# uibk-uncover/ws-unet

Hardware: AMD Instinct MI355X
Metric: 512x512 grayscale images/sec (UNet predict) (higher is better)
Workload: dtype f16 MFMA on the f16 halves + ONE block-scaled fp4 (e2m1) MFMA per tap pair for both residual cross terms (per-pixel / per-(co, tap) E8M0 scales), fp32 accumulate; planar storage

## Files before the change

### ws_unet_amd/csrc/conv3x3_q.hip

```cpp
#include "wsu_device.h"
#include <cstdlib>

namespace {

constexpr int TW = 32, TH = 16, IW = TW + 2, IH = TH + 2;
constexpr int NPIX = IW * IH;
constexpr int PLANE = NPIX * 16;
constexpr int IN_SEG = (NPIX + 63) / 64;
constexpr int S_LDS = IN_SEG * 256;
constexpr int IN_SLOT = 3 * PLANE + S_LDS;
constexpr int W_GRAN = 9 * 3 * WSU_COB * 16;
constexpr int W_SLOT = W_GRAN + 1024;
constexpr int NIN = 3, NWS = 2;
constexpr int W_BASE = NIN * IN_SLOT;
constexpr int LDS_EXTRA = W_BASE + NWS * W_SLOT;
constexpr int ZERO_BYTES = 3 * IW * 16 + 32;
constexpr int LDS_TOTAL = LDS_EXTRA + 1024 * 4 + 4 * 64 * 4 + 16 + ZERO_BYTES;
static_assert(LDS_TOTAL <= 160 * 1024 && W_SLOT % 1024 == 0, "LDS budget");
constexpr int NLOAD = 4;
constexpr int W_PIECES = W_SLOT / 1024;
constexpr unsigned OOB = 0xFFFFFFF0u;
constexpr int IN_SLOT_H = 2 * PLANE;
constexpr int W_SLOT_H = 9 * 2 * WSU_COB * 16;
template <int FMT> struct QGeo {
    static_assert(FMT == WSU_PLANAR_Q || FMT == WSU_PLANAR_H, "conv3x3_q_kernel formats: Q and H");
    static constexpr bool H = FMT == WSU_PLANAR_H;
    static constexpr int in_slot = H ? IN_SLOT_H : IN_SLOT, w_slot = H ? W_SLOT_H : W_SLOT;
    static constexpr int w_planes = H ? 2 : 3;
    static constexpr int w_base = NIN * in_slot, lds_extra = w_base + NWS * w_slot;
    static constexpr int lds_zero = lds_extra + 1024 * 4 + 4 * 64 * 4 + 16;
    static constexpr int lds_total = lds_zero + (H ? 0 : ZERO_BYTES);
    static constexpr int w_pieces = w_slot / 1024;
};
static_assert(QGeo<WSU_PLANAR_Q>::lds_zero % 16 == 0 && ZERO_BYTES % 16 == 0 && ZERO_BYTES >= 3 * IW * 16 + 16 && ZERO_BYTES >= 512 + 16, "zero block");
static_assert(QGeo<WSU_PLANAR_Q>::lds_total == LDS_TOTAL && QGeo<WSU_PLANAR_Q>::w_pieces == W_PIECES && W_SLOT_H % 1024 == 0, "LDS geometry");

struct QArgs {
    const char* x1; const char* x2; const char* wp; const float* bias;
    char* y; char* ypool;
    const float* head_w; const float* head_b; float* head_out; float* head_logit; int head_cout;
    int n, h, w, c1, c2, cout;
    int tiles_x, tiles_y, ncb, nch1, nch;
    int relu;
    int ntiles;
    unsigned* range_flag;
    int msplit;
    const float* img; const float* w1; const float* b1;
};

struct Tile { int n, y0, x0, cb, mh; };
__device__ __forceinline__ Tile tile_of(const QArgs& a, int t) {
    Tile r;
    r.cb = t % a.ncb; t /= a.ncb;
    const int tx = t % a.tiles_x; t /= a.tiles_x;
    const int ty = t % a.tiles_y;
    r.n = t / a.tiles_y; r.y0 = ty * TH; r.x0 = tx * TW;
    r.mh = 0;
    if (a.msplit) { r.mh = r.cb & 1; r.cb >>= 1; }
    return r;
}

typedef __attribute__((address_space(3))) void lds_void;
typedef __attribute__((address_space(3))) char lds_char;

__device__ __forceinline__ float dpp_xor1(float v) {
    return __builtin_bit_cast(float, __builtin_amdgcn_update_dpp(0, __builtin_bit_cast(int, v), 0xB1 , 0xF, 0xF, true));
}

template <int FMT, int LW>
__device__ __forceinline__ void q_loader(const QArgs& a, char* smem, int lane, int lw, int G, int J) {
    using Gm = QGeo<FMT>;
    constexpr int NSEG = LW < 2 ? 3 : 2;
    constexpr int NIN_OPS = (Gm::H ? 2 : 4) * NSEG;
    constexpr int W0 = Gm::H ? (LW < 2 ? LW * 3 : 6 + (LW - 2) * 6) : (LW < 2 ? LW * 5 : 10 + (LW - 2) * 9);
    constexpr int NWP = Gm::H ? (LW < 2 ? 3 : 6) : (LW < 2 ? 5 : 9);
    static_assert(2 * 5 + 2 * 9 == W_PIECES && 2 * 3 + 2 * 6 == QGeo<WSU_PLANAR_H>::w_pieces, "weight pieces over the loader waves");
    lds_char* smem3 = (lds_char*)smem;
    const unsigned hw16 = (unsigned)(a.h * a.w) * 16u;
    const unsigned chunk_bytes = Gm::H ? (unsigned)wsu_h_chunk_bytes(a.h, a.w) : (unsigned)wsu_q_chunk_bytes(a.h, a.w);
    unsigned voff[NSEG], soff[NSEG];
    auto plan = [&](const Tile& t) __attribute__((always_inline)) {
        WSU_STATIC_FOR(NSEG, k, {
            const int idx = min((LW + NLOAD * k) * 64 + lane, NPIX - 1);
            const int r = idx / IW, c = idx - r * IW;
            const int yy = wsu_reflect(t.y0 - 1 + r, a.h), xx = wsu_reflect(t.x0 - 1 + c, a.w);
            voff[k] = (unsigned)(yy * a.w + xx) * 16u;
            if constexpr (!Gm::H) soff[k] = 3u * hw16 + wsu_q_soff(yy, xx, a.tiles_x);
        });
    };
    Tile ti = tile_of(a, lw); int ci = 0, kti = 0;
    int cbw = ti.cb, cw = 0, ktw = 0;
    auto issue_in = [&](int s) __attribute__((always_inline)) {
        const char* in_src = ci < a.nch1 ? a.x1 + ((size_t)ti.n * a.nch1 + ci) * chunk_bytes : a.x2 + ((size_t)ti.n * (a.nch - a.nch1) + (ci - a.nch1)) * chunk_bytes;
        const auto rs_in = __builtin_amdgcn_make_buffer_rsrc(const_cast<char*>(in_src), 0, (int)chunk_bytes, 0x00020000);
        lds_char* slot = smem3 + (s % NIN) * Gm::in_slot;
        WSU_STATIC_FOR(NSEG, k, {
            constexpr int seg = LW + NLOAD * k;
            const bool live = seg < IN_SEG - 1 || lane < NPIX - (IN_SEG - 1) * 64;
            if (live) {
                __builtin_amdgcn_raw_ptr_buffer_load_lds(rs_in, (lds_void*)(slot + seg * 1024), 16, voff[k], 0, 0, 0);
                __builtin_amdgcn_raw_ptr_buffer_load_lds(rs_in, (lds_void*)(slot + PLANE + seg * 1024), 16, voff[k], (int)hw16, 0, 0);
                if constexpr (!Gm::H) {
                    __builtin_amdgcn_raw_ptr_buffer_load_lds(rs_in, (lds_void*)(slot + 2 * PLANE + seg * 1024), 16, voff[k], (int)(2u * hw16), 0, 0);
                    __builtin_amdgcn_raw_ptr_buffer_load_lds(rs_in, (lds_void*)(slot + 3 * PLANE + seg * 256), 1, soff[k], 0, 0, 0);
                }
            }
        });
        if (++ci == a.nch && s + 1 < J) { ci = 0; ++kti; ti = tile_of(a, lw + kti * G); plan(ti); }
    };
    auto issue_w = [&](int s) __attribute__((always_inline)) {
        const auto rs_w = __builtin_amdgcn_make_buffer_rsrc(const_cast<char*>(a.wp), 0, 0x7FFFFFF0, 0x00020000);
        const int w_base = (cbw * a.nch + cw) * Gm::w_slot;
        lds_char* slot = smem3 + Gm::w_base + (s % NWS) * Gm::w_slot;
        WSU_STATIC_FOR(NWP, k, {
            constexpr int piece = W0 + k;
            __builtin_amdgcn_raw_ptr_buffer_load_lds(rs_w, (lds_void*)(slot + piece * 1024), 16, (unsigned)lane * 16u, w_base + piece * 1024, 0, 0);
        });
        if (++cw == a.nch && s + 1 < J) { cw = 0; ++ktw; cbw = tile_of(a, lw + ktw * G).cb; }
    };
    if (J <= 0) return;
    plan(ti);
    issue_w(0);
    issue_in(0);
    if (J > 1) issue_in(1);
    if (J > 1) asm volatile("s_waitcnt vmcnt(%0)" :: "n"(NIN_OPS) : "memory"); else asm volatile("s_waitcnt vmcnt(0)" ::: "memory");
    for (int j = 0; ; ++j) {
        __builtin_amdgcn_s_barrier();
        asm volatile("" ::: "memory");
        if (j + 1 >= J) break;
        issue_w(j + 1);
        const bool more = j + 2 < J;
        if (more) issue_in(j + 2);
        if (more) asm volatile("s_waitcnt vmcnt(%0)" :: "n"(NIN_OPS) : "memory"); else asm volatile("s_waitcnt vmcnt(0)" ::: "memory");
    }
}

__device__ __forceinline__ void q_loader_f1(const QArgs& a, char* smem, int lane, int lw, int G, int J, int lw8) {
    if (J <= 0) return;
    lds_char* smem3 = (lds_char*)smem;
    constexpr int F1_PX = 3;
    float pimg[F1_PX][9];
    float f1_max = 0.f;
    Tile ti = tile_of(a, lw); int ci = 0, kti = 0;
    int cbw = ti.cb, cw = 0, ktw = 0;
    auto window = [&](const Tile& tt) __attribute__((always_inline)) {
        const float* img = a.img + (size_t)tt.n * a.h * a.w;
#pragma unroll
        for (int k = 0; k < F1_PX; ++k) {
            const int idx = min((lw8 + NLOAD * k) * 64 + lane, NPIX - 1);
            const int r = idx / IW, cc = idx - r * IW;
            const int yy = wsu_reflect(tt.y0 - 1 + r, a.h), xx = wsu_reflect(tt.x0 - 1 + cc, a.w);
#pragma unroll
            for (int tp = 0; tp < 9; ++tp)
                pimg[k][tp] = img[(size_t)wsu_reflect(yy + tp / 3 - 1, a.h) * a.w + wsu_reflect(xx + tp % 3 - 1, a.w)];
        }
    };
    typedef __attribute__((address_space(4))) const f32x2 cst_f32x2;
    auto compute_in = [&](int s) __attribute__((always_inline)) {
        char* slot = smem + (s % NIN) * IN_SLOT;
        cst_f32x2* wt = (cst_f32x2*)(a.w1 + ci * 16);
        cst_f32x2* bt = (cst_f32x2*)(a.b1 + ci * 16);
        f32x2 acc[F1_PX][8];
#pragma unroll
        for (int g = 0; g < 8; ++g) {
            const f32x2 b = bt[g];
#pragma unroll
            for (int k = 0; k < F1_PX; ++k) acc[k][g] = b;
        }
#pragma unroll
        for (int tp = 0; tp < 9; ++tp) {
            f32x2 wv[8];
#pragma unroll
            for (int g = 0; g < 8; ++g) wv[g] = wt[tp * 32 + g];
#pragma unroll
            for (int k = 0; k < F1_PX; ++k) {
                const f32x2 pw = {pimg[k][tp & ~1], pimg[k][(tp | 1) < 9 ? (tp | 1) : tp]};
#pragma unroll
                for (int g = 0; g < 8; ++g) {
                    if (tp & 1) asm volatile("v_pk_fma_f32 %0, %1, %2, %0 op_sel:[1,0,0] op_sel_hi:[1,1,1]" : "+v"(acc[k][g]) : "v"(pw), "s"(wv[g]));
                    else asm volatile("v_pk_fma_f32 %0, %1, %2, %0 op_sel:[0,0,0] op_sel_hi:[0,1,1]" : "+v"(acc[k][g]) : "v"(pw), "s"(wv[g]));
                }
            }
        }
        asm volatile("s_nop 0" ::: "memory");
#pragma unroll
        for (int k = 0; k < F1_PX; ++k) {
            const int idx = (lw8 + NLOAD * k) * 64 + lane;
            f32x4 v[4];
#pragma unroll
            for (int g = 0; g < 4; ++g) v[g] = mk_f4(acc[k][2 * g][0], acc[k][2 * g][1], acc[k][2 * g + 1][0], acc[k][2 * g + 1][1]);
#pragma unroll
            for (int g = 0; g < 4; ++g)
#pragma unroll
                for (int e = 0; e < 4; ++e) { v[g][e] = fmaxf(v[g][e], 0.f); f1_max = fmaxf(f1_max, v[g][e]); }
            u32x4 h0, h1, qg; uint32_t sb;
            wsu_q4_encode16(v, h0, h1, qg, sb);
            if (lw8 + NLOAD * k < IN_SEG && idx < NPIX) {
                char* d = slot + idx * 16;
                *reinterpret_cast<u32x4*>(d) = h0;
                *reinterpret_cast<u32x4*>(d + PLANE) = h1;
                *reinterpret_cast<u32x4*>(d + 2 * PLANE) = qg;
                *reinterpret_cast<uint32_t*>(slot + 3 * PLANE + idx * 4) = sb;
            }
        }
        if (++ci == a.nch && s + 1 < J) { ci = 0; ++kti; ti = tile_of(a, lw + kti * G); window(ti); }
    };
    const int w0 = lw8 < 2 ? lw8 * 5 : 10 + (lw8 - 2) * 9, nwp = lw8 < 2 ? 5 : 9;
    auto issue_w = [&](int s) __attribute__((always_inline)) {
        const auto rs_w = __builtin_amdgcn_make_buffer_rsrc(const_cast<char*>(a.wp), 0, 0x7FFFFFF0, 0x00020000);
        const int w_base = (cbw * a.nch + cw) * W_SLOT;
        lds_char* slot = smem3 + W_BASE + (s % NWS) * W_SLOT;
#pragma unroll
        for (int k = 0; k < 9; ++k)
            if (k < nwp)
                __builtin_amdgcn_raw_ptr_buffer_load_lds(rs_w, (lds_void*)(slot + (w0 + k) * 1024), 16, (unsigned)lane * 16u, w_base + (w0 + k) * 1024, 0, 0);
        if (++cw == a.nch && s + 1 < J) { cw = 0; ++ktw; cbw = tile_of(a, lw + ktw * G).cb; }
    };
    window(ti);
    issue_w(0);
    compute_in(0);
    if (J > 1) compute_in(1);
    asm volatile("s_waitcnt vmcnt(0) lgkmcnt(0)" ::: "memory");
    for (int j = 0; ; ++j) {
        __builtin_amdgcn_s_barrier();
        asm volatile("" ::: "memory");
        if (j + 1 >= J) break;
        issue_w(j + 1);
        if (j + 2 < J) compute_in(j + 2);
        asm volatile("s_waitcnt vmcnt(0) lgkmcnt(0)" ::: "memory");
    }
    if (a.range_flag && __builtin_amdgcn_ballot_w64(!(f1_max <= WSU_F8_RANGE)) != 0 && lane == 0) atomicOr(a.range_flag, 1u);
}

template <int RQ, int HC, bool POOL, bool FQ, bool MSPLIT, bool F1 = false, int FMT = WSU_PLANAR_Q>
__global__ __launch_bounds__((16 / RQ + NLOAD) * 64) __attribute__((amdgpu_waves_per_eu(RQ == 4 ? 2 : 3, RQ == 4 ? 2 : 3)))
void conv3x3_q_kernel(const QArgs a) {
    using Gm = QGeo<FMT>;
    constexpr bool H = Gm::H;
    static_assert(!(H && F1), "the fused first layer computes Q inputs");
    constexpr int NWAVE = 16 / RQ, NT = (NWAVE + NLOAD) * 64;
    extern __shared__ __attribute__((aligned(16))) char smem[];
    const int tid = threadIdx.x;
    const int wv = __builtin_amdgcn_readfirstlane(tid >> 6), lane = tid & 63, l31 = lane & 31, hh = lane >> 5;
    const int l31_k = l31, hh_k = hh;
    const int G = gridDim.x;
    const int lw = (int)wsu_xcd_remap(blockIdx.x, G);
    const int K = a.ntiles > lw ? (a.ntiles - lw + G - 1) / G : 0;
    const int J = K * a.nch;

    float* s_bias = reinterpret_cast<float*>(smem + Gm::lds_extra);
    float* s_hw = s_bias + 1024;
    float* s_hb = s_hw + 4 * 64;
    for (int i = tid; i < a.cout; i += NT) s_bias[i] = a.bias ? a.bias[i] : 0.f;
    constexpr bool HEAD = HC > 0;
    if constexpr (HEAD) {
        for (int i = tid; i < a.head_cout * 64; i += NT) s_hw[i] = a.head_w[i];
        if (tid < 4) s_hb[tid] = (a.head_b && tid < a.head_cout) ? a.head_b[tid] : 0.f;
    }
    if constexpr (!Gm::H) {
        for (int i = tid; i < ZERO_BYTES / 4; i += NT) reinterpret_cast<unsigned*>(smem + Gm::lds_zero)[i] = 0u;
        asm volatile("s_waitcnt lgkmcnt(0)" ::: "memory");
    }

    if (wv >= NWAVE) {
        if constexpr (F1) { q_loader_f1(a, smem, lane, lw, G, J, wv - NWAVE); return; }
        switch (wv - NWAVE) {
            case 0: q_loader<FMT, 0>(a, smem, lane, lw, G, J); break;
            case 1: q_loader<FMT, 1>(a, smem, lane, lw, G, J); break;
            case 2: q_loader<FMT, 2>(a, smem, lane, lw, G, J); break;
            default: q_loader<FMT, 3>(a, smem, lane, lw, G, J); break;
        }
        return;
    }

    Tile cur = tile_of(a, lw);
    constexpr int MH = MSPLIT ? 1 : 2;
    constexpr bool PIPE = !H;
    constexpr bool EPO = !MSPLIT && HC == 0 && RQ != 4;
    f32x16 acc[2][4];
    int kt = 0, j = 0;
    unsigned q_in_off = 0, q_w_off = Gm::w_base;
    unsigned nx_in = 0, nx_w = Gm::w_base;
    unsigned a_off = 0, b_off = 0, x_w = 0, x_w4 = 0, x_sa = 0, x_sa4 = 0, x_b1 = 0, x_b2 = 0, x_b4 = 0, x_sb0 = 0, x_sb1 = 0, x_sb2 = 0;
    constexpr unsigned W4_IMM = (unsigned)((8 * 3 + 2) * 64) * 16u, B4_IMM = (unsigned)(2 * IW + 2) * 16u;
    typedef __attribute__((address_space(3))) const unsigned char lds_cuchar;
    typedef __attribute__((address_space(3))) const int lds_cint;
    typedef __attribute__((address_space(3))) const u32x4 lds_cu32x4;
    const unsigned Lb = (unsigned)(size_t)(lds_char*)smem;
    auto at = [](unsigned addr) __attribute__((always_inline)) { return (lds_char*)(size_t)addr; };
    auto begin_step = [&]() __attribute__((always_inline)) {
        q_in_off = nx_in; q_w_off = nx_w;
        nx_in = nx_in + (unsigned)Gm::in_slot == (unsigned)(NIN * Gm::in_slot) ? 0u : nx_in + (unsigned)Gm::in_slot;
        static_assert(NWS == 2, "nx_w toggles between the two weight slots the loaders fill as s % NWS");
        nx_w = (unsigned)(2 * Gm::w_base + Gm::w_slot) - nx_w;
        a_off = Lb + q_w_off + (unsigned)((cur.mh * 32 + l31) * 16) + (unsigned)(hh * 64 * 16);
        b_off = Lb + q_in_off + (unsigned)(((RQ * wv) * IW + l31) * 16) + (unsigned)(hh * PLANE);
        if constexpr (!H) {
            unsigned hq = (unsigned)hh;
            asm volatile("" : "+v"(hq));
            const unsigned zero = Lb + (unsigned)Gm::lds_zero;
            const unsigned w0 = Lb + q_w_off + (unsigned)(cur.mh * 32 + l31) * 16u;
            const unsigned p0 = Lb + q_in_off + 2 * PLANE + (unsigned)((RQ * wv) * IW + l31) * 16u;
            x_w = w0 + hq * (unsigned)(3 * 64 * 16);
            x_w4 = hq ? zero - W4_IMM : w0;
            x_sa4 = Lb + q_w_off + W_GRAN + (unsigned)(cur.mh * 32 + l31);
            x_sa = x_sa4 + hq * 64u;
            x_b1 = p0 + hq * 16u;
            x_b2 = p0 + hq * (unsigned)((IW - 2) * 16);
            x_b4 = hq ? zero - B4_IMM : p0;
            x_sb0 = Lb + q_in_off + 3 * PLANE + (unsigned)((RQ * wv) * IW + l31) * 4u;
            x_sb1 = x_sb0 + hq * 4u;
            x_sb2 = x_sb0 + hq * (unsigned)((IW - 2) * 4);
            asm volatile("" : "+v"(a_off), "+v"(b_off), "+v"(x_w), "+v"(x_w4), "+v"(x_sa), "+v"(x_sa4));
            asm volatile("" : "+v"(x_b1), "+v"(x_b2), "+v"(x_b4), "+v"(x_sb0), "+v"(x_sb1), "+v"(x_sb2));
        } else {
            asm volatile("" : "+v"(a_off), "+v"(b_off));
        }
        __builtin_amdgcn_s_barrier();
        asm volatile("" ::: "memory");
    };
    auto zero_acc = [&]() __attribute__((always_inline)) {
#pragma unroll
        for (int m = 0; m < MH; ++m)
#pragma unroll
            for (int q = 0; q < RQ; ++q)
#pragma unroll
                for (int r = 0; r < 16; ++r) acc[m][q][r] = 0.f;
    };
    auto main_term = [&](auto tap_c, auto ms_c, auto first_c) __attribute__((always_inline)) {
        constexpr int tap = decltype(tap_c)::value, dy = tap / 3, dx = tap % 3;
        constexpr int ms = decltype(ms_c)::value, ML = ms < 0 ? 0 : ms, MU = ms < 0 ? MH : ms + 1;
        constexpr bool FIRST = decltype(first_c)::value;
        u32x4 ah[2], bh[4];
_Pragma("unroll")
        for (int m = ML; m < MU; ++m) ah[m] = *(lds_cu32x4*)(at(a_off) + ((tap * Gm::w_planes) * 64 + m * 32) * 16);
_Pragma("unroll")
        for (int q = 0; q < RQ; ++q) bh[q] = *(lds_cu32x4*)(at(b_off) + ((q + dy) * IW + dx) * 16);
_Pragma("unroll")
        for (int m = ML; m < MU; ++m)
_Pragma("unroll")
            for (int q = 0; q < RQ; ++q) {
                if constexpr (FIRST) acc[m][q] = wsu_mfma_f16_z(ah[m], bh[q]);
                else wsu_mfma_f16(ah[m], bh[q], acc[m][q]);
            }
    };
    auto q4_reads = [&](auto tp_c, auto ml_c, auto mu_c, u32x4* a4, u32x4* b4, int* sa, int* sb) __attribute__((always_inline)) {
        constexpr int tp = decltype(tp_c)::value, ML = decltype(ml_c)::value, MU = decltype(mu_c)::value;
        constexpr bool single = 2 * tp + 1 >= 9;
        constexpr int t0 = 2 * tp, pix0 = (t0 / 3) * IW + t0 % 3;
        constexpr unsigned wimm = (unsigned)((6 * tp + 2) * 64) * 16u;
        static_assert(!single || (wimm == W4_IMM && (unsigned)pix0 * 16u == B4_IMM), "tap 8");
        const unsigned wbase = single ? x_w4 : x_w, sabase = single ? x_sa4 : x_sa;
        const unsigned bbase = single ? x_b4 : (tp == 1 ? x_b2 : x_b1), sbbase = single ? x_sb0 : (tp == 1 ? x_sb2 : x_sb1);
_Pragma("unroll")
        for (int m = ML; m < MU; ++m) {
            a4[m] = *(lds_cu32x4*)(at(wbase) + wimm + m * 32 * 16);
            sa[m] = *(lds_cuchar*)(at(sabase) + 128 * tp + m * 32);
        }
_Pragma("unroll")
        for (int q = 0; q < RQ; ++q) {
            b4[q] = *(lds_cu32x4*)(at(bbase) + (pix0 + q * IW) * 16);
            sb[q] = *(lds_cint*)(at(sbbase) + (pix0 + q * IW) * 4);
        }
    };
    auto cross_q4 = [&](auto tp_c, auto ms_c, auto first_c) __attribute__((always_inline)) {
        constexpr int ms = decltype(ms_c)::value, ML = ms < 0 ? 0 : ms, MU = ms < 0 ? MH : ms + 1;
        constexpr bool FIRST = decltype(first_c)::value;
        u32x4 a4[2], b4[4]; int sa[2], sb[4];
        q4_reads(tp_c, std::integral_constant<int, ML>{}, std::integral_constant<int, MU>{}, a4, b4, sa, sb);
_Pragma("unroll")
        for (int m = ML; m < MU; ++m)
_Pragma("unroll")
            for (int q = 0; q < RQ; ++q) {
                if constexpr (FIRST) acc[m][q] = wsu_mfma_q4_z(a4[m], b4[q], sa[m], sb[q]);
                else wsu_mfma_q4(a4[m], b4[q], sa[m], sb[q], acc[m][q]);
            }
    };
    constexpr std::false_type not_first{};
    constexpr std::true_type tile_first{};
    auto units_range = [&](auto ms_c, auto lo_c, auto hi_c, auto first_c) __attribute__((always_inline)) {
        constexpr int lo = decltype(lo_c)::value, hi = decltype(hi_c)::value;
        constexpr bool FIRST = decltype(first_c)::value;
        static_assert(!FIRST || lo == 0, "a tile opens with tap pair 0");
        WSU_STATIC_FOR(hi - lo, i, {
            constexpr int tp = lo + i;
            if constexpr (!H) cross_q4(std::integral_constant<int, tp>{}, ms_c, std::integral_constant<bool, FIRST && tp == 0>{});
            main_term(std::integral_constant<int, 2 * tp>{}, ms_c, std::integral_constant<bool, FIRST && H && tp == 0>{});
            if constexpr (2 * tp + 1 < 9) main_term(std::integral_constant<int, 2 * tp + 1>{}, ms_c, not_first);
        });
    };
    constexpr std::integral_constant<int, -1> all_m{};
    struct Frag { u32x4 a[2]; u32x4 b[4]; int sa[2]; int sb[4]; };
    auto load_unit = [&](auto u_c, Frag& f, u32x4* row1) __attribute__((always_inline)) {
        constexpr int u = decltype(u_c)::value, tp = u / 3, k = u % 3;
        if constexpr (k == 0) {
            q4_reads(std::integral_constant<int, tp>{}, std::integral_constant<int, 0>{}, std::integral_constant<int, MH>{}, f.a, f.b, f.sa, f.sb);
        } else {
            constexpr int tap = 2 * tp + k - 1, dy = tap / 3, dx = tap % 3;
_Pragma("unroll")
            for (int m = 0; m < MH; ++m) f.a[m] = *(lds_cu32x4*)(at(a_off) + ((tap * 3) * 64 + m * 32) * 16);
            if constexpr (RQ == 2) {
                if constexpr (dy > 0) f.b[0] = row1[tap - 3];
                else f.b[0] = *(lds_cu32x4*)(at(b_off) + (dy * IW + dx) * 16);
                f.b[1] = row1[tap] = *(lds_cu32x4*)(at(b_off) + ((1 + dy) * IW + dx) * 16);
            } else {
_Pragma("unroll")
                for (int q = 0; q < RQ; ++q) f.b[q] = *(lds_cu32x4*)(at(b_off) + ((q + dy) * IW + dx) * 16);
            }
        }
    };
    auto mma_unit = [&](auto u_c, Frag& f, auto first_c) __attribute__((always_inline)) {
        constexpr int u = decltype(u_c)::value, k = u % 3;
        constexpr bool FIRST = decltype(first_c)::value && u == 0;
        if constexpr (k == 0) {
_Pragma("unroll")
            for (int m = 0; m < MH; ++m)
_Pragma("unroll")
                for (int q = 0; q < RQ; ++q) {
                    if constexpr (FIRST) acc[m][q] = wsu_mfma_q4_z(f.a[m], f.b[q], f.sa[m], f.sb[q]);
                    else wsu_mfma_q4(f.a[m], f.b[q], f.sa[m], f.sb[q], acc[m][q]);
                }
        } else {
_Pragma("unroll")
            for (int m = 0; m < MH; ++m)
_Pragma("unroll")
                for (int q = 0; q < RQ; ++q) wsu_mfma_f16(f.a[m], f.b[q], acc[m][q]);
        }
    };
    auto units_pipelined = [&](auto first_c) __attribute__((always_inline)) {
        constexpr int NU = 14;
        Frag fr[2];
        u32x4 row1[9];
        load_unit(std::integral_constant<int, 0>{}, fr[0], row1);
        WSU_STATIC_FOR(NU, u, {
            if constexpr (u + 1 < NU) load_unit(std::integral_constant<int, u + 1>{}, fr[(u + 1) % 2], row1);
            __builtin_amdgcn_sched_barrier(0);
            mma_unit(u_c, fr[u % 2], first_c);
            __builtin_amdgcn_sched_barrier(0);
        });
    };
    auto units_all = [&](auto ms_c, auto first_c) __attribute__((always_inline)) {
        if constexpr (PIPE && decltype(ms_c)::value < 0) { units_pipelined(first_c); return; }
        units_range(ms_c, std::integral_constant<int, 0>{}, std::integral_constant<int, 5>{}, first_c);
    };

    auto finish_tile = [&]() __attribute__((always_inline)) {
        int l31 = l31_k, hh = hh_k;
        asm volatile("" : "+v"(l31), "+v"(hh));
        const int col = cur.x0 + l31;
        const unsigned hw16 = (unsigned)(a.h * a.w) * 16u;
        const int nco = a.cout >> 4;
        float hz[4][HC > 0 ? HC : 1];
        float vmax = 0.f;
        const float relu_floor = a.relu ? 0.f : -__builtin_inff();
#pragma unroll
        for (int q = 0; q < RQ; ++q)
#pragma unroll
            for (int o = 0; o < (HC > 0 ? HC : 1); ++o) hz[q][o] = 0.f;
        struct QOff { unsigned g0, g1, q, s; };
        auto pair_off = [&](unsigned plane_bytes, unsigned off0, unsigned off1, unsigned soff0, unsigned soff1, bool ok0, bool ok1) __attribute__((always_inline)) {
            const unsigned hp = hh ? plane_bytes : 0u;
            const bool okm = hh ? ok1 : ok0;
            QOff o = {ok0 ? off0 + hp : OOB, ok1 ? off1 + hp : OOB, okm ? (hh ? off1 : off0) + 2u * plane_bytes : OOB, okm ? 3u * plane_bytes + (hh ? soff1 : soff0) : OOB};
            asm volatile("" : "+v"(o.g0), "+v"(o.g1), "+v"(o.q), "+v"(o.s));
            return o;
        };
        constexpr bool YQ = FQ && !H;
        QOff qo[RQ / 2] = {}, qop = {};
        if constexpr (YQ) {
            const unsigned sblk = (unsigned)(((cur.y0 >> 4) * a.tiles_x + (cur.x0 >> 5)) * 512);
_Pragma("unroll")
            for (int rp = 0; rp < RQ / 2; ++rp) {
                const int r0 = RQ * wv + 2 * rp, row0 = cur.y0 + r0;
                qo[rp] = pair_off(hw16, (unsigned)(row0 * a.w + col) * 16u, (unsigned)((row0 + 1) * a.w + col) * 16u,
                                  sblk + (unsigned)(r0 * 32 + l31), sblk + (unsigned)((r0 + 1) * 32 + l31), row0 < a.h && col < a.w, row0 + 1 < a.h && col < a.w);
            }
            if constexpr (POOL) {
                const int hp = a.h >> 1, wp2 = a.w >> 1, ptx = (wp2 + 31) >> 5;
                const int gy0 = (cur.y0 >> 1) + (RQ / 2) * wv, gx = (cur.x0 >> 1) + (l31 >> 1);
                const unsigned php16 = (unsigned)(hp * wp2) * 16u;
                if constexpr (RQ == 4) {
                    const bool okx = !(l31 & 1) && gx < wp2;
                    qop = pair_off(php16, (unsigned)(gy0 * wp2 + gx) * 16u, (unsigned)((gy0 + 1) * wp2 + gx) * 16u,
                                   wsu_q_soff(gy0, gx, ptx), wsu_q_soff(gy0 + 1, gx, ptx), okx && gy0 < hp, okx && gy0 + 1 < hp);
                } else {
                    const unsigned coff = (l31 & 1) ? (unsigned)wsu_q_chunk_bytes(hp, wp2) : 0u;
                    const unsigned off = (unsigned)(gy0 * wp2 + gx) * 16u + coff, soff = wsu_q_soff(gy0, gx, ptx) + coff;
                    const bool ok = gx < wp2 && gy0 < hp;
                    qop = {ok ? off + (hh ? php16 : 0u) : OOB, OOB, (ok && !hh) ? off + 2u * php16 : OOB, (ok && !hh) ? 3u * php16 + soff : OOB};
                    asm volatile("" : "+v"(qop.g0), "+v"(qop.q), "+v"(qop.s));
                }
            }
        }
        auto store_pair_q = [&](const f32x4& X0, const f32x4& Y0, const f32x4& X1, const f32x4& Y1, char* base, unsigned chunk_bytes, const QOff& o, bool have, bool fold) __attribute__((always_inline)) {
            u32x4 g0, g1; uint32_t dh0, dr0, sb0, dh1, dr1, sb1;
            const float mx0 = wsu_q4_pre(X0, Y0, g0, dh0, dr0, sb0);
            const float mx1 = wsu_q4_pre(X1, Y1, g1, dh1, dr1, sb1);
            if (fold) vmax = wsu_max3(vmax, mx0, mx1);
            const u32x4 qg = wsu_q4_pair(dh0, dr0, dh1, dr1);
            const auto rs = __builtin_amdgcn_make_buffer_rsrc(base, 0, have ? (int)chunk_bytes : 0, 0x00020000);
            __builtin_amdgcn_raw_buffer_store_b128(g0, rs, (int)o.g0, 0, 0);
            __builtin_amdgcn_raw_buffer_store_b128(g1, rs, (int)o.g1, 0, 0);
            __builtin_amdgcn_raw_buffer_store_b128(qg, rs, (int)o.q, 0, 0);
            __builtin_amdgcn_raw_buffer_store_b8((unsigned char)(hh ? sb1 : sb0), rs, (int)o.s, 0, 0);
        };
        auto store_one_q = [&](const f32x4& X, const f32x4& Y, char* base, unsigned chunk_bytes, const QOff& o) __attribute__((always_inline)) {
            u32x4 g; uint32_t dh, dr, sb;
            wsu_q4_pre(X, Y, g, dh, dr, sb);
            const u32x4 qg = wsu_q4_single(dh, dr);
            const auto rs = __builtin_amdgcn_make_buffer_rsrc(base, 0, (int)chunk_bytes, 0x00020000);
            __builtin_amdgcn_raw_buffer_store_b128(g, rs, (int)o.g0, 0, 0);
            __builtin_amdgcn_raw_buffer_store_b128(qg, rs, (int)o.q, 0, 0);
            __builtin_amdgcn_raw_buffer_store_b8((unsigned char)sb, rs, (int)o.s, 0, 0);
        };
        auto store_one_h = [&](const f32x4& X, const f32x4& Y, char* base, unsigned plane_bytes, unsigned off, bool ok, bool have) __attribute__((always_inline)) {
            const auto rs = __builtin_amdgcn_make_buffer_rsrc(base, 0, have ? (int)(2u * plane_bytes) : 0, 0x00020000);
            __builtin_amdgcn_raw_buffer_store_b128(wsu_h_granule(X, Y), rs, (int)(ok ? off + (hh ? plane_bytes : 0u) : OOB), 0, 0);
        };
        auto store_one_a = [&](const f32x4& X, const f32x4& Y, char* base, unsigned plane_bytes, unsigned off, bool ok, bool have) __attribute__((always_inline)) {
            uint32_t xh0, xh1, xlo, yh0, yh1, ylo;
            wsu_split4_f16r8(X, WSU_F8_XLO_DIV, xh0, xh1, xlo);
            wsu_split4_f16r8(Y, WSU_F8_XLO_DIV, yh0, yh1, ylo);
            wsu_swap32(xh0, yh0); wsu_swap32(xh1, yh1);
            uint32_t xlp = xlo, ylp = ylo;
            wsu_swap32(xlo, xlp); wsu_swap32(ylo, ylp);
            const auto rs = __builtin_amdgcn_make_buffer_rsrc(base, 0, have ? (int)(3u * plane_bytes) : 0, 0x00020000);
            __builtin_amdgcn_raw_buffer_store_b128(mk_u4(xh0, xh1, yh0, yh1), rs, (int)(ok ? off + (hh ? plane_bytes : 0u) : OOB), 0, 0);
            __builtin_amdgcn_raw_buffer_store_b128(mk_u4(xlo, xlp, ylo, ylp), rs, (int)((ok && !hh) ? off + 2u * plane_bytes : OOB), 0, 0);
        };
        auto epi_m = [&](auto m_c, auto&& hook) __attribute__((always_inline)) {
            constexpr int m = decltype(m_c)::value;
            constexpr int NH = RQ / 2;
            f32x4 spx, spy;
            auto piece = [&](auto cp_c) __attribute__((always_inline)) {
                constexpr int cp = decltype(cp_c)::value;
                const int oc = cur.cb * 4 + (m + cur.mh) * 2 + cp;
                const int co0 = oc * 16 + 4 * hh;
                const bool have_y = a.y != nullptr;
                f32x4 px[2], py[2];
                WSU_STATIC_FOR(RQ / 2, rp, {
                    hook(std::integral_constant<int, NH * cp + rp>{});
                    f32x4 vx[2], vy[2];
                    const f32x4 bx = *reinterpret_cast<const f32x4*>(s_bias + co0), by = *reinterpret_cast<const f32x4*>(s_bias + co0 + 8);
_Pragma("unroll")
                    for (int u = 0; u < 2; ++u) {
_Pragma("unroll")
                        for (int e = 0; e < 4; ++e) {
                            const float x = fmaxf(acc[m][2 * rp + u][8 * cp + e] + bx[e], relu_floor), y = fmaxf(acc[m][2 * rp + u][8 * cp + 4 + e] + by[e], relu_floor);
                            vx[u][e] = x; vy[u][e] = y;
                            if constexpr (H || !FQ) vmax = fmaxf(fmaxf(vmax, fabsf(x)), fabsf(y));
                        }
                    }
                    if constexpr (HEAD) {
                        const int lc = (m * 2 + cp) * 16 + 4 * hh;
_Pragma("unroll")
                        for (int o = 0; o < HC; ++o)
                            if (HC == 1 || o < a.head_cout)
_Pragma("unroll")
                                for (int u = 0; u < 2; ++u)
_Pragma("unroll")
                                    for (int e = 0; e < 4; ++e)
                                        hz[2 * rp + u][o] = fmaf(vx[u][e], s_hw[o * 64 + lc + e], fmaf(vy[u][e], s_hw[o * 64 + lc + 8 + e], hz[2 * rp + u][o]));
                    }
                    const int r0 = RQ * wv + 2 * rp, row0 = cur.y0 + r0;
                    if (!HEAD || have_y) {
                        if constexpr (H) {
                            char* base = a.y + ((size_t)cur.n * nco + oc) * (2u * hw16);
                            WSU_STATIC_FOR(2, u, {
                                store_one_h(vx[u], vy[u], base, hw16, (unsigned)((row0 + u) * a.w + col) * 16u, row0 + u < a.h && col < a.w, have_y);
                            });
                        } else if constexpr (FQ) {
                            const unsigned cb_ = (unsigned)wsu_q_chunk_bytes(a.h, a.w);
                            char* base = a.y + ((size_t)cur.n * nco + oc) * cb_;
                            store_pair_q(vx[0], vy[0], vx[1], vy[1], base, cb_, qo[rp], have_y, true);
                        } else {
                            char* base = a.y + (((size_t)cur.n * nco + oc) * 3) * hw16;
                            WSU_STATIC_FOR(2, u, {
                                store_one_a(vx[u], vy[u], base, hw16, (unsigned)((row0 + u) * a.w + col) * 16u, row0 + u < a.h && col < a.w, have_y);
                            });
                        }
                    }
                    if constexpr (POOL) {
_Pragma("unroll")
                        for (int e = 0; e < 4; ++e) {
                            const float cx = fmaxf(vx[0][e], vx[1][e]), cy = fmaxf(vy[0][e], vy[1][e]);
                            px[rp][e] = fmaxf(cx, dpp_xor1(cx)); py[rp][e] = fmaxf(cy, dpp_xor1(cy));
                        }
                    }
                });
                if constexpr (POOL) {
                    const int hp = a.h >> 1, wp2 = a.w >> 1;
                    const int gy0 = (cur.y0 >> 1) + (RQ / 2) * wv, gx = (cur.x0 >> 1) + (l31 >> 1);
                    const bool okx = !(l31 & 1) && gx < wp2;
                    const unsigned php16 = (unsigned)(hp * wp2) * 16u;
                    if constexpr (H) {
                        char* base = a.ypool + ((size_t)cur.n * nco + oc) * (2u * php16);
#pragma unroll
                        for (int rp = 0; rp < RQ / 2; ++rp)
                            store_one_h(px[rp], py[rp], base, php16, (unsigned)((gy0 + rp) * wp2 + gx) * 16u, okx && gy0 + rp < hp, true);
                    } else if constexpr (FQ) {
                        const unsigned cbp = (unsigned)wsu_q_chunk_bytes(hp, wp2);
                        char* base = a.ypool + ((size_t)cur.n * nco + oc) * cbp;
                        if constexpr (RQ == 4) {
                            store_pair_q(px[0], py[0], px[1], py[1], base, cbp, qop, true, false);
                        } else if constexpr (cp == 0) {
                            spx = px[0]; spy = py[0];
                        } else {
                            static_assert(cp == 1, "piece 1 closes the pair: its chunk follows piece 0's");
                            const bool odd = (l31 & 1) != 0;
                            f32x4 sx, sy;
_Pragma("unroll")
                            for (int e = 0; e < 4; ++e) { sx[e] = odd ? px[0][e] : spx[e]; sy[e] = odd ? py[0][e] : spy[e]; }
                            store_one_q(sx, sy, base - cbp, 2u * cbp, qop);
                        }
                    } else {
                        char* base = a.ypool + (((size_t)cur.n * nco + oc) * 3) * php16;
#pragma unroll
                        for (int rp = 0; rp < RQ / 2; ++rp)
                            store_one_a(px[rp], py[rp], base, php16, (unsigned)((gy0 + rp) * wp2 + gx) * 16u, okx && gy0 + rp < hp, true);
                    }
                }
            };
            piece(std::integral_constant<int, 0>{});
            piece(std::integral_constant<int, 1>{});
        };
        auto nothing = [](auto) __attribute__((always_inline)) {};
        if constexpr (EPO) {
            constexpr int NHT = 2 * (RQ / 2);
            epi_m(std::integral_constant<int, 0>{}, [&](auto h_c) __attribute__((always_inline)) {
                constexpr int h = decltype(h_c)::value;
                constexpr int lo = 5 * h / NHT, hi = 5 * (h + 1) / NHT;
                if constexpr (hi > lo) units_range(std::integral_constant<int, 1>{}, std::integral_constant<int, lo>{}, std::integral_constant<int, hi>{}, not_first);
            });
            epi_m(std::integral_constant<int, 1>{}, nothing);
        } else {
            WSU_STATIC_FOR(MH, m, { (void)m; epi_m(m_c, nothing); });
        }
        if constexpr (HEAD) {
            const size_t hw = (size_t)a.h * a.w;
#pragma unroll
            for (int q = 0; q < RQ; ++q) {
                const int row = cur.y0 + RQ * wv + q;
#pragma unroll
                for (int o = 0; o < HC; ++o)
                    if (HC == 1 || o < a.head_cout) {
                        uint32_t mine = __builtin_bit_cast(uint32_t, hz[q][o]), other = mine;
                        wsu_swap32(mine, other);
                        const float z = __builtin_bit_cast(float, mine) + __builtin_bit_cast(float, other) + s_hb[o];
                        if (!hh && row < a.h && col < a.w) {
                            const size_t plane = ((size_t)cur.n * a.head_cout + o) * hw;
                            const uint32_t off = (uint32_t)(row * a.w + col);
                            if (a.head_logit) (a.head_logit + plane)[off] = z;
                            (a.head_out + plane)[off] = 1.f / (1.f + expf(-z));
                        }
                    }
            }
        }
        if (a.range_flag && (a.y || POOL) && __builtin_amdgcn_ballot_w64(!(vmax <= (H ? WSU_F16_RANGE : WSU_F8_RANGE))) != 0 && lane == 0)
            atomicOr(a.range_flag, 1u);
        ++kt;
        if (j + 1 < J) cur = tile_of(a, lw + kt * G);
    };
    for (int t = 0; t < K; ++t) {
        if (a.nch == 1) {
            zero_acc();
        } else {
            begin_step(); units_all(all_m, tile_first); ++j;
            for (int cc = 2; cc < a.nch; ++cc) { begin_step(); units_all(all_m, not_first); ++j; }
        }
        begin_step();
        if constexpr (EPO) units_all(std::integral_constant<int, 0>{}, not_first);
        else units_all(all_m, not_first);
        __builtin_amdgcn_sched_barrier(0);
        finish_tile();
        ++j;
    }
}

__global__ void pack_conv3x3_f4_kernel(const float* __restrict__ w, char* __restrict__ dst, int cin, int cout) {
    const int nch = cin / 16;
    const long long total = (long long)(cout / WSU_COB) * nch * 9 * WSU_COB;
    for (long long d = (long long)blockIdx.x * blockDim.x + threadIdx.x; d < total; d += (long long)gridDim.x * blockDim.x) {
        long long t = d;
        const int co = (int)(t % WSU_COB); t /= WSU_COB;
        const int tap = (int)(t % 9); t /= 9;
        const int c = (int)(t % nch); const int cb = (int)(t / nch);
        float v[16], r[16];
        uint32_t h[8];
#pragma unroll
        for (int e = 0; e < 16; ++e) v[e] = w[(((size_t)(cb * WSU_COB + co) * cin + c * 16 + e) * 3 + tap / 3) * 3 + tap % 3];
#pragma unroll
        for (int e = 0; e < 8; ++e) {
            const _Float16 a = (_Float16)v[2 * e], b = (_Float16)v[2 * e + 1];
            h[e] = (uint32_t)__builtin_bit_cast(unsigned short, a) | ((uint32_t)__builtin_bit_cast(unsigned short, b) << 16);
            r[2 * e] = (v[2 * e] - (float)a) * 2048.f; r[2 * e + 1] = (v[2 * e + 1] - (float)b) * 2048.f;
        }
        const u32x4 h0 = mk_u4(h[0], h[1], h[2], h[3]), h1 = mk_u4(h[4], h[5], h[6], h[7]);
        const int E = wsu_q4_block_exp(wsu_f16x16_max_abs_bits(h0, h1));
        const float sc = wsu_pow2f(E);
        uint32_t q[4] = {0, 0, 0, 0};
        WSU_STATIC_FOR(8, e, { q[e >> 2] = __builtin_amdgcn_cvt_scalef32_pk_fp4_f32(q[e >> 2], r[2 * e], r[2 * e + 1], sc, e & 3); });
        q[2] = wsu_f16x8_to_fp4(h0, sc); q[3] = wsu_f16x8_to_fp4(h1, sc);
        char* slice = dst + ((size_t)cb * nch + c) * W_SLOT;
        char* base = slice + (size_t)(tap * 3) * (WSU_COB * 16) + co * 16;
        *reinterpret_cast<u32x4*>(base) = h0;
        *reinterpret_cast<u32x4*>(base + WSU_COB * 16) = h1;
        *reinterpret_cast<u32x4*>(base + 2 * WSU_COB * 16) = mk_u4(q[0], q[1], q[2], q[3]);
        slice[W_GRAN + tap * 64 + co] = (char)(E + 127 - 11);
        if (tap == 0 && co < 7) *reinterpret_cast<u32x4*>(slice + W_GRAN + 576 + co * 64) = mk_u4(0, 0, 0, 0), *reinterpret_cast<u32x4*>(slice + W_GRAN + 576 + co * 64 + 16) = mk_u4(0, 0, 0, 0),
            *reinterpret_cast<u32x4*>(slice + W_GRAN + 576 + co * 64 + 32) = mk_u4(0, 0, 0, 0), *reinterpret_cast<u32x4*>(slice + W_GRAN + 576 + co * 64 + 48) = mk_u4(0, 0, 0, 0);
    }
}

__global__ void pack_conv3x3_h_kernel(const float* __restrict__ w, char* __restrict__ dst, int cin, int cout) {
    const int nch = cin / 16;
    const long long total = (long long)(cout / WSU_COB) * nch * 9 * WSU_COB;
    for (long long d = (long long)blockIdx.x * blockDim.x + threadIdx.x; d < total; d += (long long)gridDim.x * blockDim.x) {
        long long t = d;
        const int co = (int)(t % WSU_COB); t /= WSU_COB;
        const int tap = (int)(t % 9); t /= 9;
        const int c = (int)(t % nch); const int cb = (int)(t / nch);
        uint32_t h[8];
#pragma unroll
        for (int e = 0; e < 8; ++e) {
            const size_t i0 = (((size_t)(cb * WSU_COB + co) * cin + c * 16 + 2 * e) * 3 + tap / 3) * 3 + tap % 3;
            const _Float16 a = (_Float16)w[i0], b = (_Float16)w[i0 + 9];
            h[e] = (uint32_t)__builtin_bit_cast(unsigned short, a) | ((uint32_t)__builtin_bit_cast(unsigned short, b) << 16);
        }
        char* base = dst + ((size_t)cb * nch + c) * W_SLOT_H + (size_t)(tap * 2) * (WSU_COB * 16) + co * 16;
        *reinterpret_cast<u32x4*>(base) = mk_u4(h[0], h[1], h[2], h[3]);
        *reinterpret_cast<u32x4*>(base + WSU_COB * 16) = mk_u4(h[4], h[5], h[6], h[7]);
    }
}

#define WSU_Q_VARIANTS_RQ(X, RQ)                    \
    X(RQ, 0, false, false, false, false, WSU_PLANAR_Q) \
    X(RQ, 0, false, true, false, false, WSU_PLANAR_Q)  \
    X(RQ, 0, true, false, false, false, WSU_PLANAR_Q)  \
    X(RQ, 0, true, true, false, false, WSU_PLANAR_Q)   \
    X(RQ, 1, false, false, false, false, WSU_PLANAR_Q) \
    X(RQ, 4, false, false, false, false, WSU_PLANAR_Q) \
    X(RQ, 0, false, false, true, false, WSU_PLANAR_Q)  \
    X(RQ, 0, false, true, true, false, WSU_PLANAR_Q)
#define WSU_Q_VARIANTS(X)                            \
    WSU_Q_VARIANTS_RQ(X, 4)                          \
    WSU_Q_VARIANTS_RQ(X, 2)                          \
    X(2, 0, true, true, false, true, WSU_PLANAR_Q)   \
    X(2, 0, false, true, false, false, WSU_PLANAR_H) \
    X(2, 0, true, true, false, false, WSU_PLANAR_H)  \
    X(2, 1, false, true, false, false, WSU_PLANAR_H) \
    X(2, 4, false, true, false, false, WSU_PLANAR_H) \
    X(2, 0, false, true, true, false, WSU_PLANAR_H)
#define WSU_Q_INST(RQ, HC, POOL, FQ, MSPLIT, F1, FMT) template __global__ void conv3x3_q_kernel<RQ, HC, POOL, FQ, MSPLIT, F1, FMT>(const QArgs);
WSU_Q_VARIANTS(WSU_Q_INST)

struct QVariant {
    int rq, hc; bool pool, fq, msplit, f1; int fmt;
    void (*kernel)(const QArgs);
    bool raised;
};
#define WSU_Q_ROW(RQ, HC, POOL, FQ, MSPLIT, F1, FMT) {RQ, HC, POOL, FQ, MSPLIT, F1, FMT, conv3x3_q_kernel<RQ, HC, POOL, FQ, MSPLIT, F1, FMT>, false},
QVariant q_variants[] = {WSU_Q_VARIANTS(WSU_Q_ROW)};

int q_launch(QArgs a, const char* who, int fmt, int rq, bool yq, bool msplit_on, hipStream_t s) {
    const bool h = fmt == WSU_PLANAR_H, f1 = a.img != nullptr;
    const int ncu = wsu_cu_count(who);
    if (!ncu) return WSU_ERR_HIP;
    const int hc = !a.head_w ? 0 : (a.head_cout == 1 ? 1 : 4);
    const bool pool = a.ypool != nullptr, fq = h || (yq && !hc);
    a.msplit = !f1 && msplit_on && !hc && !pool && 2 * (long long)a.ntiles <= ncu;
    if (a.msplit) { a.ncb *= 2; a.ntiles *= 2; }
    for (QVariant& v : q_variants) {
        if (v.rq != rq || v.hc != hc || v.pool != pool || v.fq != fq || v.msplit != (a.msplit != 0) || v.f1 != f1 || v.fmt != fmt) continue;
        const int lds = h ? QGeo<WSU_PLANAR_H>::lds_total : LDS_TOTAL;
        if (!v.raised) {
            if (int rc = wsu_raise_lds(v.kernel, lds, f1 ? "conv3x3_q<F1>" : (h ? "conv3x3_q<H>" : "conv3x3_q"))) return rc;
            v.raised = true;
        }
        hipLaunchKernelGGL(v.kernel, dim3(a.ntiles < ncu ? a.ntiles : ncu), dim3((16 / rq + NLOAD) * 64), lds, s, a);
        return wsu_check_launch(f1 ? "conv3x3_q_kernel<F1>" : (h ? (a.msplit ? "conv3x3_q_kernel<H, msplit>" : "conv3x3_q_kernel<H>")
                                                                 : (a.msplit ? "conv3x3_q_kernel<msplit>" : "conv3x3_q_kernel")));
    }
    wsu_set_error("%s: no kernel variant for this combination of outputs", who);
    return WSU_ERR_UNSUPPORTED;
}

int q_args(QArgs& a, const char* who, const void* x1, const void* x2, const float* img, const float* w1, const float* b1, const void* wp, const float* bias,
           void* y, void* y_pool, const float* head_w, const float* head_b, float* head_out, float* head_logit, int head_cout,
           int n, int h, int w, int c1, int c2, int cout, int relu, int y_format, unsigned formats, const char* formats_msg, unsigned* range_flag) {
    const bool f1 = img || w1 || b1;
    WSU_REQUIRE(wp && (f1 ? img && w1 && b1 && y && y_pool : x1 && (y || y_pool || head_w)), "%s: null pointer", who);
    WSU_REQUIRE(!f1 || (((uintptr_t)w1 & 63) == 0 && ((uintptr_t)b1 & 63) == 0), "%s: w1_taps and b1 must be 64-byte aligned (scalar 16-dword loads)", who);
    WSU_REQUIRE(y_format >= 0 && y_format < 32 && ((formats >> y_format) & 1u), "%s: y_format must be %s", who, formats_msg);
    WSU_REQUIRE(n > 0 && h >= 2 && w >= 2, "%s: bad shape n=%d h=%d w=%d (reflect pad 1 needs h,w >= 2)", who, n, h, w);
    WSU_REQUIRE(c1 > 0 && c1 % 16 == 0 && c2 >= 0 && c2 % 16 == 0 && (c2 == 0) == (x2 == nullptr), "%s: c1=%d c2=%d must be multiples of 16", who, c1, c2);
    WSU_REQUIRE(cout > 0 && cout % WSU_COB == 0 && cout <= 1024, "%s: cout=%d must be a multiple of %d (<= 1024)", who, cout, WSU_COB);
    WSU_REQUIRE(!head_w || (head_out && cout == WSU_COB && head_cout >= 1 && head_cout <= 4), "%s: fused head needs cout == %d and 1..4 head planes", who, WSU_COB);
    WSU_REQUIRE(!y_pool || (h % 2 == 0 && w % 2 == 0), "%s: fused pool needs even h, w (got h=%d w=%d)", who, h, w);
    WSU_REQUIRE(!(y_pool && head_w), "%s: the fused pool and the fused head exclude each other", who);
    WSU_REQUIRE(!(head_w && y && y_format == WSU_PLANAR_Q), "%s: a y beside the fused head is written in format WSU_PLANAR_A", who);
    WSU_REQUIRE((long long)h * w * 50 < 0xFFFFFFF0LL, "%s: h*w too large (a chunk must stay below 4 GiB)", who);
    a.x1 = (const char*)x1; a.x2 = (const char*)x2; a.wp = (const char*)wp; a.bias = bias;
    a.y = (char*)y; a.ypool = (char*)y_pool;
    a.head_w = head_w; a.head_b = head_b; a.head_out = head_out; a.head_logit = head_logit; a.head_cout = head_cout;
    a.range_flag = range_flag;
    a.n = n; a.h = h; a.w = w; a.c1 = c1; a.c2 = c2; a.cout = cout;
    a.tiles_x = (w + TW - 1) / TW; a.tiles_y = (h + TH - 1) / TH; a.ncb = cout / WSU_COB;
    a.nch1 = c1 / 16; a.nch = (c1 + c2) / 16; a.relu = relu; a.msplit = 0;
    a.img = img; a.w1 = w1; a.b1 = b1;
    const long long nt = (long long)n * a.tiles_x * a.tiles_y * a.ncb;
    WSU_REQUIRE(nt > 0 && nt < 0x3FFFFFFFLL, "%s: %lld tiles out of range", who, nt);
    a.ntiles = (int)nt;
    return WSU_OK;
}

bool q_msplit_on() {
    static const int on = [] { const char* e = getenv("WSU_PL_MSPLIT"); return e ? atoi(e) : 1; }();
    return on != 0;
}

size_t packed_bytes(int cin, int cout, int slot) {
    if (cin <= 0 || cout <= 0 || cin % 16 || cout % WSU_COB) return 0;
    return (size_t)(cout / WSU_COB) * (cin / 16) * slot;
}
int pack(void (*kernel)(const float*, char*, int, int), const char* who, const char* kernel_name, const float* w_oihw, void* w_packed, int cin, int cout, void* stream) {
    WSU_REQUIRE(w_oihw && w_packed, "%s: null pointer", who);
    WSU_REQUIRE(cin > 0 && cin % 16 == 0 && cout > 0 && cout % WSU_COB == 0, "%s: cin=%d must be a multiple of 16, cout=%d of %d", who, cin, cout, WSU_COB);
    hipLaunchKernelGGL(kernel, dim3(512), dim3(256), 0, static_cast<hipStream_t>(stream), w_oihw, (char*)w_packed, cin, cout);
    return wsu_check_launch(kernel_name);
}

}

extern "C" {

size_t wsu_conv3x3_packed_f4_bytes(int cin, int cout) { return packed_bytes(cin, cout, W_SLOT); }
int wsu_conv3x3_pack_f4(const float* w_oihw, void* w_packed, int cin, int cout, void* stream) {
    return pack(pack_conv3x3_f4_kernel, "conv3x3_pack_f4", "pack_conv3x3_f4_kernel", w_oihw, w_packed, cin, cout, stream);
}

int wsu_conv3x3_q_fused_first_fwd(const float* img, const float* w1_taps, const float* b1, const void* w_packed_f4, const float* bias, void* y, void* y_pool,
                                  int n, int h, int w, int cout, int relu, unsigned* range_flag, void* stream) {
    const char* who = "conv3x3_q_fused_first";
    WSU_REQUIRE(img && w1_taps && b1, "%s: null pointer", who);
    QArgs a;
    if (int rc = q_args(a, who, nullptr, nullptr, img, w1_taps, b1, w_packed_f4, bias, y, y_pool, nullptr, nullptr, nullptr, nullptr, 0,
                        n, h, w, 64, 0, cout, relu, WSU_PLANAR_Q, 1u << WSU_PLANAR_Q, "WSU_PLANAR_Q", range_flag)) return rc;
    return q_launch(a, who, WSU_PLANAR_Q, 2, true, false, static_cast<hipStream_t>(stream));
}

size_t wsu_planar_q_bytes(int n, int c, int h, int w) {
    if (n <= 0 || c <= 0 || c % 16 || h <= 0 || w <= 0) return 0;
    return (size_t)n * (size_t)(c / 16) * wsu_q_chunk_bytes(h, w);
}

int wsu_conv3x3_q_fwd(const void* x1, const void* x2, const void* w_packed_f4, const float* bias, void* y, void* y_pool,
                      const float* head_w, const float* head_b, float* head_out, float* head_logit, int head_cout,
                      int n, int h, int w, int c1, int c2, int cout, int relu, int y_format, unsigned* range_flag, void* stream) {
    QArgs a;
    if (int rc = q_args(a, "conv3x3_q", x1, x2, nullptr, nullptr, nullptr, w_packed_f4, bias, y, y_pool, head_w, head_b, head_out, head_logit, head_cout,
                        n, h, w, c1, c2, cout, relu, y_format, 1u << WSU_PLANAR_A | 1u << WSU_PLANAR_Q, "WSU_PLANAR_A or WSU_PLANAR_Q", range_flag)) return rc;
    static const int rq = [] { const char* e = getenv("WSU_Q_ROWS"); return (e && atoi(e) == 4) ? 4 : 2; }();
    return q_launch(a, "conv3x3_q", WSU_PLANAR_Q, rq, y_format == WSU_PLANAR_Q, q_msplit_on(), static_cast<hipStream_t>(stream));
}

size_t wsu_planar_h_bytes(int n, int c, int h, int w) {
    if (n <= 0 || c <= 0 || c % 16 || h <= 0 || w <= 0) return 0;
    return (size_t)n * (size_t)(c / 16) * wsu_h_chunk_bytes(h, w);
}

size_t wsu_conv3x3_packed_h_bytes(int cin, int cout) { return packed_bytes(cin, cout, W_SLOT_H); }
int wsu_conv3x3_pack_h(const float* w_oihw, void* w_packed, int cin, int cout, void* stream) {
    return pack(pack_conv3x3_h_kernel, "conv3x3_pack_h", "pack_conv3x3_h_kernel", w_oihw, w_packed, cin, cout, stream);
}

int wsu_conv3x3_h_fwd(const void* x1, const void* x2, const void* w_packed_h, const float* bias, void* y, void* y_pool,
                      const float* head_w, const float* head_b, float* head_out, float* head_logit, int head_cout,
                      int n, int h, int w, int c1, int c2, int cout, int relu, int y_format, unsigned* range_flag, void* stream) {
    QArgs a;
    if (int rc = q_args(a, "conv3x3_h", x1, x2, nullptr, nullptr, nullptr, w_packed_h, bias, y, y_pool, head_w, head_b, head_out, head_logit, head_cout,
                        n, h, w, c1, c2, cout, relu, y_format, 1u << WSU_PLANAR_H, "WSU_PLANAR_H", range_flag)) return rc;
    return q_launch(a, "conv3x3_h", WSU_PLANAR_H, 2, true, q_msplit_on(), static_cast<hipStream_t>(stream));
}

}
```

### ws_unet_amd/csrc/conv3x3_qu.hip

```cpp
#include "wsu_device.h"

namespace {

constexpr int TW = 32, TH = 16;
constexpr int CW = 17, CH = 9, CPIX = CW * CH;
constexpr int NPIX_S = 4 * CPIX;
constexpr int PLANE_S = NPIX_S * 16;
constexpr int SEG_S = (NPIX_S + 63) / 64;
constexpr int IN_S = 3 * PLANE_S + SEG_S * 256;
constexpr int LP = 33, LH = TH / 2 + 2, LW_ = TW / 2 + 2;
constexpr int NPIX_L = LP * LH;
constexpr int PLANE_L = NPIX_L * 16;
constexpr int SEG_L = (NPIX_L + 63) / 64;
constexpr int IN_L = 3 * PLANE_L + SEG_L * 256;
constexpr int W_GRAN_S = 9 * 3 * WSU_COB * 16;
constexpr int W_S = W_GRAN_S + 1024;
constexpr int W_UNITS_L = 8;
constexpr int W_GRAN_L = W_UNITS_L * 3 * WSU_COB * 16;
constexpr int W_L = W_GRAN_L + 1024;
constexpr int PIECES_S = W_S / 1024, PIECES_L = W_L / 1024;
constexpr int REGION = 80640;
constexpr int OFF_SW = IN_S, OFF_LIN = W_L, OFF_LW1 = W_L + IN_L;
constexpr int LDS_BIAS = 2 * REGION;
constexpr int MAX_COUT = 512;
constexpr int LDS_TOTAL = LDS_BIAS + MAX_COUT * 4;
static_assert(IN_S + W_S <= REGION && OFF_LW1 + W_L <= REGION && (REGION & 0xF) == 0 && LDS_TOTAL <= 160 * 1024, "LDS budget");
static_assert((OFF_SW | OFF_LIN | OFF_LW1) % 16 == 0, "16-byte aligned allocations");
constexpr int ZERO_BYTES = 576;
constexpr int LDS_ZERO = 2 * REGION - ZERO_BYTES;
static_assert(IN_S + W_S <= REGION - ZERO_BYTES && OFF_LW1 + W_L <= REGION - ZERO_BYTES && LDS_ZERO % 16 == 0 && ZERO_BYTES >= 2 * CW * 16 + 16 + 16, "zero block");
constexpr int NLOAD = 4, NWAVE = 8, NT = (NWAVE + NLOAD) * 64;
constexpr unsigned OOB = 0xFFFFFFF0u;
constexpr int W_S_H = 9 * 2 * WSU_COB * 16;
constexpr int W_L_H = W_UNITS_L * 2 * WSU_COB * 16;
constexpr int PIECES_S_H = W_S_H / 1024, PIECES_L_H = W_L_H / 1024;

struct UArgs {
    const char* xl; const char* xs; const char* wps; const char* wpl; const float* bias;
    char* y;
    int n, h, w, hl, wl, cl, c2, cout;
    int tiles_x, tiles_y, ltiles_x, ncb, nchS, nchL;
    int relu, ntiles;
    unsigned* range_flag;
};

struct Tile { int n, y0, x0, cb; };
__device__ __forceinline__ Tile tile_of(const UArgs& a, int t) {
    Tile r;
    r.cb = t % a.ncb; t /= a.ncb;
    const int tx = t % a.tiles_x; t /= a.tiles_x;
    const int ty = t % a.tiles_y;
    r.n = t / a.tiles_y; r.y0 = ty * TH; r.x0 = tx * TW;
    return r;
}

typedef __attribute__((address_space(3))) void lds_void;
typedef __attribute__((address_space(3))) char lds_char;

__device__ __forceinline__ void wait_vm(int n) {
#define WSU_VM_CASE(k) case k: asm volatile("s_waitcnt vmcnt(" #k ")" ::: "memory"); break;
    switch (n) {
        WSU_VM_CASE(0) WSU_VM_CASE(1) WSU_VM_CASE(2) WSU_VM_CASE(3) WSU_VM_CASE(4) WSU_VM_CASE(5) WSU_VM_CASE(6) WSU_VM_CASE(7) WSU_VM_CASE(8) WSU_VM_CASE(9)
        WSU_VM_CASE(10) WSU_VM_CASE(11) WSU_VM_CASE(12) WSU_VM_CASE(13) WSU_VM_CASE(14) WSU_VM_CASE(15) WSU_VM_CASE(16) WSU_VM_CASE(17) WSU_VM_CASE(18) WSU_VM_CASE(19)
        WSU_VM_CASE(20) WSU_VM_CASE(21) WSU_VM_CASE(22) WSU_VM_CASE(23) WSU_VM_CASE(24) WSU_VM_CASE(25) WSU_VM_CASE(26) WSU_VM_CASE(27) WSU_VM_CASE(28) WSU_VM_CASE(29)
        WSU_VM_CASE(30) WSU_VM_CASE(31) WSU_VM_CASE(32) WSU_VM_CASE(33) WSU_VM_CASE(34) WSU_VM_CASE(35) WSU_VM_CASE(36) WSU_VM_CASE(37) WSU_VM_CASE(38) WSU_VM_CASE(39)
        default: asm volatile("s_waitcnt vmcnt(0)" ::: "memory"); break;
    }
#undef WSU_VM_CASE
}


template <int FMT, int LW>
__device__ __forceinline__ void u_loader(const UArgs& a, char* smem, int lane, int lw, int G, int K) {
    constexpr bool H = FMT == WSU_PLANAR_H;
    constexpr int NSS = LW < 2 ? 3 : 2;
    constexpr int NSL = LW < 2 ? 2 : 1;
    constexpr int OPS_INS = (H ? 2 : 4) * NSS, OPS_INL = (H ? 2 : 4) * NSL;
    constexpr int WS0 = H ? (LW < 2 ? LW * 3 : 6 + (LW - 2) * 6) : (LW < 2 ? LW * 5 : 10 + (LW - 2) * 9);
    constexpr int NWS = H ? (LW < 2 ? 3 : 6) : (LW < 2 ? 5 : 9);
    constexpr int WL0 = H ? (LW < 2 ? LW * 3 : 6 + (LW - 2) * 5) : (LW < 2 ? LW * 5 : (LW == 2 ? 10 : 17));
    constexpr int NWL = H ? (LW < 2 ? 3 : 5) : (LW < 2 ? 5 : (LW == 2 ? 7 : 8));
    constexpr int WSLICE_S = H ? W_S_H : W_S, WSLICE_L = H ? W_L_H : W_L;
    static_assert(2 * 5 + 2 * 9 == PIECES_S && 2 * 5 + 7 + 8 == PIECES_L, "weight pieces over the loader waves");
    static_assert(2 * 3 + 2 * 6 == PIECES_S_H && 2 * 3 + 2 * 5 == PIECES_L_H, "weight pieces over the loader waves (format H)");
    lds_char* smem3 = (lds_char*)smem;
    const unsigned hw16 = (unsigned)(a.h * a.w) * 16u, hwl16 = (unsigned)(a.hl * a.wl) * 16u;
    const unsigned cbytes_s = H ? (unsigned)wsu_h_chunk_bytes(a.h, a.w) : (unsigned)wsu_q_chunk_bytes(a.h, a.w);
    const unsigned cbytes_l = H ? (unsigned)wsu_h_chunk_bytes(a.hl, a.wl) : (unsigned)wsu_q_chunk_bytes(a.hl, a.wl);
    const int T = a.nchS + a.nchL;
    const int J = K * T;
    if (J <= 0) return;
    unsigned voS[NSS], soS[NSS], voL[NSL], soL[NSL];
    auto plan = [&](const Tile& t) __attribute__((always_inline)) {
        WSU_STATIC_FOR(NSS, k, {
            const int idx = min((LW + NLOAD * k) * 64 + lane, NPIX_S - 1);
            const int p = idx / CPIX, rem = idx - p * CPIX;
            const int lr = rem / CW, lc = rem - lr * CW;
            const int yy = wsu_reflect(t.y0 - 1 + 2 * lr + (p >> 1), a.h), xx = wsu_reflect(t.x0 - 1 + 2 * lc + (p & 1), a.w);
            voS[k] = (unsigned)(yy * a.w + xx) * 16u;
            if constexpr (!H) soS[k] = 3u * hw16 + wsu_q_soff(yy, xx, a.tiles_x);
        });
        WSU_STATIC_FOR(NSL, k, {
            const int idx = min((LW + NLOAD * k) * 64 + lane, NPIX_L - 1);
            const int r = idx / LP, c = min(idx - r * LP, LW_ - 1);
            const int yy = min(max((t.y0 >> 1) - 1 + r, 0), a.hl - 1), xx = min(max((t.x0 >> 1) - 1 + c, 0), a.wl - 1);
            voL[k] = (unsigned)(yy * a.wl + xx) * 16u;
            if constexpr (!H) soL[k] = 3u * hwl16 + wsu_q_soff(yy, xx, a.ltiles_x);
        });
    };
    int a_kt = 0, a_c = 0, a_r = 0; bool a_low = false;
    Tile at = tile_of(a, lw);
    unsigned region = 0;
    auto issue_alloc = [&](lds_char* slot) __attribute__((always_inline)) {
        int nops;
        const bool is_in = a_low ? a_r == 1 : a_r == 0;
        if (is_in && !a_low) {
            const char* src = a.xs + ((size_t)at.n * a.nchS + a_c) * cbytes_s;
            const auto rs = __builtin_amdgcn_make_buffer_rsrc(const_cast<char*>(src), 0, (int)cbytes_s, 0x00020000);
            WSU_STATIC_FOR(NSS, k, {
                constexpr int seg = LW + NLOAD * k;
                if (seg < SEG_S - 1 || lane < NPIX_S - (SEG_S - 1) * 64) {
                    __builtin_amdgcn_raw_ptr_buffer_load_lds(rs, (lds_void*)(slot + seg * 1024), 16, voS[k], 0, 0, 0);
                    __builtin_amdgcn_raw_ptr_buffer_load_lds(rs, (lds_void*)(slot + PLANE_S + seg * 1024), 16, voS[k], (int)hw16, 0, 0);
                    if constexpr (!H) {
                        __builtin_amdgcn_raw_ptr_buffer_load_lds(rs, (lds_void*)(slot + 2 * PLANE_S + seg * 1024), 16, voS[k], (int)(2u * hw16), 0, 0);
                        __builtin_amdgcn_raw_ptr_buffer_load_lds(rs, (lds_void*)(slot + 3 * PLANE_S + seg * 256), 1, soS[k], 0, 0, 0);
                    }
                }
            });
            nops = OPS_INS;
        } else if (is_in) {
            const char* src = a.xl + ((size_t)at.n * a.nchL + a_c) * cbytes_l;
            const auto rs = __builtin_amdgcn_make_buffer_rsrc(const_cast<char*>(src), 0, (int)cbytes_l, 0x00020000);
            WSU_STATIC_FOR(NSL, k, {
                constexpr int seg = LW + NLOAD * k;
                if (seg < SEG_L - 1 || lane < NPIX_L - (SEG_L - 1) * 64) {
                    __builtin_amdgcn_raw_ptr_buffer_load_lds(rs, (lds_void*)(slot + seg * 1024), 16, voL[k], 0, 0, 0);
                    __builtin_amdgcn_raw_ptr_buffer_load_lds(rs, (lds_void*)(slot + PLANE_L + seg * 1024), 16, voL[k], (int)hwl16, 0, 0);
                    if constexpr (!H) {
                        __builtin_amdgcn_raw_ptr_buffer_load_lds(rs, (lds_void*)(slot + 2 * PLANE_L + seg * 1024), 16, voL[k], (int)(2u * hwl16), 0, 0);
                        __builtin_amdgcn_raw_ptr_buffer_load_lds(rs, (lds_void*)(slot + 3 * PLANE_L + seg * 256), 1, soL[k], 0, 0, 0);
                    }
                }
            });
            nops = OPS_INL;
        } else if (!a_low) {
            const auto rs = __builtin_amdgcn_make_buffer_rsrc(const_cast<char*>(a.wps), 0, 0x7FFFFFF0, 0x00020000);
            const int base = (at.cb * a.nchS + a_c) * WSLICE_S;
            WSU_STATIC_FOR(NWS, k, {
                constexpr int piece = WS0 + k;
                __builtin_amdgcn_raw_ptr_buffer_load_lds(rs, (lds_void*)(slot + piece * 1024), 16, (unsigned)lane * 16u, base + piece * 1024, 0, 0);
            });
            nops = NWS;
        } else {
            const auto rs = __builtin_amdgcn_make_buffer_rsrc(const_cast<char*>(a.wpl), 0, 0x7FFFFFF0, 0x00020000);
            const int base = ((at.cb * a.nchL + a_c) * 2 + (a_r == 2 ? 1 : 0)) * WSLICE_L;
            WSU_STATIC_FOR(NWL, k, {
                constexpr int piece = WL0 + k;
                __builtin_amdgcn_raw_ptr_buffer_load_lds(rs, (lds_void*)(slot + piece * 1024), 16, (unsigned)lane * 16u, base + piece * 1024, 0, 0);
            });
            nops = NWL;
        }
        return nops;
    };
    auto issue_step = [&]() __attribute__((always_inline)) {
        lds_char* base = smem3 + region;
        int nops;
        if (!a_low) {
            a_r = 0; nops = issue_alloc(base);
            a_r = 1; nops += issue_alloc(base + OFF_SW);
            if (++a_c == a.nchS) { a_c = 0; a_low = true; }
        } else {
            a_r = 0; nops = issue_alloc(base);
            a_r = 1; nops += issue_alloc(base + OFF_LIN);
            a_r = 2; nops += issue_alloc(base + OFF_LW1);
            if (++a_c == a.nchL) {
                a_low = false; a_c = 0;
                if (++a_kt < K) { at = tile_of(a, lw + a_kt * G); plan(at); }
            }
        }
        region ^= (unsigned)REGION;
        return nops;
    };
    plan(at);
    {
        issue_step();
        const int n1 = J > 1 ? issue_step() : 0;
        wait_vm(n1);
    }
    for (int j = 0; ; ++j) {
        __builtin_amdgcn_s_barrier();
        asm volatile("" ::: "memory");
        if (j + 1 >= J) break;
        if (j >= 1) issue_step();
        wait_vm(0);
    }
}

template <int FMT>
__global__ __launch_bounds__(NT) __attribute__((amdgpu_waves_per_eu(3, 3)))
void conv3x3_qu_kernel(const UArgs a) {
    constexpr bool H = FMT == WSU_PLANAR_H;
    constexpr int WPL = H ? 2 : 3;
    extern __shared__ __attribute__((aligned(16))) char smem[];
    const int tid = threadIdx.x;
    const int wv = __builtin_amdgcn_readfirstlane(tid >> 6), lane = tid & 63;
    const int G = gridDim.x;
    const int lw = (int)wsu_xcd_remap(blockIdx.x, G);
    const int K = a.ntiles > lw ? (a.ntiles - lw + G - 1) / G : 0;
    float* s_bias = reinterpret_cast<float*>(smem + LDS_BIAS);
    for (int i = tid; i < a.cout; i += NT) s_bias[i] = a.bias ? a.bias[i] : 0.f;
    if constexpr (!H) {
        for (int i = tid; i < ZERO_BYTES / 4; i += NT) reinterpret_cast<unsigned*>(smem + LDS_ZERO)[i] = 0u;
        asm volatile("s_waitcnt lgkmcnt(0)" ::: "memory");
    }

    if (wv >= NWAVE) {
        switch (wv - NWAVE) {
            case 0: u_loader<FMT, 0>(a, smem, lane, lw, G, K); break;
            case 1: u_loader<FMT, 1>(a, smem, lane, lw, G, K); break;
            case 2: u_loader<FMT, 2>(a, smem, lane, lw, G, K); break;
            default: u_loader<FMT, 3>(a, smem, lane, lw, G, K); break;
        }
        return;
    }

    const int cls = wv & 3, py = cls >> 1, px = cls & 1, rh = wv >> 2;
    const int l31 = lane & 31, hh = lane >> 5;
    const int lrow = l31 >> 4, lcol = lrow ? ((l31 + 15) & 15) : l31;
    const unsigned laneS = (unsigned)(((4 * rh + lrow) * CW + lcol) * 16), laneL = (unsigned)(((4 * rh + lrow) * LP + lcol) * 16);
    constexpr unsigned QS = 2 * CW * 16, QL = 2 * LP * 16;
    Tile cur = tile_of(a, lw);
    f32x16 acc[2][2];
    unsigned region = 0;
    unsigned in_off = 0, w_off = 0;
    auto next_region = [&]() __attribute__((always_inline)) { const unsigned r = region; region ^= (unsigned)REGION; return r; };
    int hh_q = hh;
    typedef __attribute__((address_space(3))) const unsigned char lds_cuchar;
    typedef __attribute__((address_space(3))) const int lds_cint;
    typedef __attribute__((address_space(3))) const u32x4 lds_cu32x4;
    lds_char* L = (lds_char*)smem;
    const unsigned Lb = (unsigned)(size_t)L;
    auto at = [](unsigned addr) __attribute__((always_inline)) { return (lds_char*)(size_t)addr; };
    auto tap_s = [&](int ky, int kx) __attribute__((always_inline)) {
        return (unsigned)(((((py + ky) & 1) * 2 + ((px + kx) & 1)) * CPIX + ((py + ky) >> 1) * CW + ((px + kx) >> 1)) * 16);
    };
    unsigned a_off = 0, b_off = 0, hd_w = 0, hd_sa = 0, hd_b = 0, hd_sb = 0, x_w = 0, x_w4 = 0, x_sa = 0, x_sa4 = 0, x_b4 = 0;
    constexpr unsigned W4_IMM = (unsigned)((8 * 3 + 2) * 64) * 16u;
    unsigned tap_sel[5] = {};
    if constexpr (!H) {
        WSU_STATIC_FOR(5, tp, {
            constexpr int t0 = 2 * tp, t1 = (2 * tp + 1 < 9) ? 2 * tp + 1 : 2 * tp;
            tap_sel[tp] = ((hh ? tap_s(t1 / 3, t1 % 3) : tap_s(t0 / 3, t0 % 3)) + laneS) >> 2;
            asm volatile("" : "+v"(tap_sel[tp]));
        });
    }
    auto sync_step = [&](auto low_c) __attribute__((always_inline)) {
        constexpr bool LOW = decltype(low_c)::value;
        const unsigned r = next_region();
        in_off = LOW ? r + OFF_LIN : r;
        w_off = LOW ? r : r + OFF_SW;
        hh_q = hh;
        asm volatile("" : "+v"(hh_q));
        a_off = Lb + w_off + (unsigned)l31 * 16u + (unsigned)hh * 1024u;
        b_off = Lb + in_off + (unsigned)hh * (LOW ? PLANE_L : PLANE_S) + (LOW ? laneL : laneS);
        if constexpr (!H && !LOW) {
            const unsigned hq = (unsigned)hh_q, zero = Lb + (unsigned)LDS_ZERO;
            const unsigned w0 = Lb + w_off + (unsigned)l31 * 16u;
            x_w = w0 + hq * (unsigned)(3 * 64 * 16);
            x_w4 = hq ? zero - W4_IMM : w0;
            x_sa4 = Lb + w_off + W_GRAN_S + (unsigned)l31;
            x_sa = x_sa4 + hq * 64u;
            hd_b = Lb + in_off + 2 * PLANE_S + tap_sel[0] * 4u;
            hd_sb = Lb + in_off + 3 * PLANE_S + tap_sel[0];
            x_b4 = hq ? zero : Lb + in_off + 2 * PLANE_S + tap_sel[4] * 4u;
            asm volatile("" : "+v"(a_off), "+v"(b_off), "+v"(x_w), "+v"(x_w4), "+v"(x_sa), "+v"(x_sa4), "+v"(hd_b), "+v"(hd_sb), "+v"(x_b4));
        } else if constexpr (!H) {
            const int u = cls * 2 + hh_q;
            const unsigned pb = (unsigned)((py * LP + px) * 16) + (unsigned)hh_q * 16u + laneL;
            hd_w = Lb + w_off + (unsigned)((u * 3 + 2) * 64 + l31) * 16u;
            hd_sa = Lb + w_off + W_GRAN_L + (unsigned)(u * 64 + l31);
            hd_b = Lb + in_off + 2 * PLANE_L + pb;
            hd_sb = Lb + in_off + 3 * PLANE_L + (pb >> 2);
            asm volatile("" : "+v"(a_off), "+v"(b_off), "+v"(hd_w), "+v"(hd_sa), "+v"(hd_b), "+v"(hd_sb));
        } else {
            asm volatile("" : "+v"(a_off), "+v"(b_off));
        }
        __builtin_amdgcn_s_barrier();
        asm volatile("" ::: "memory");
    };
    struct Frag { u32x4 a[2]; u32x4 b[2]; int sa[2]; int sb[2]; };
    auto load_unit = [&](auto u_c, Frag& f) __attribute__((always_inline)) {
        constexpr int u = decltype(u_c)::value, tp = u / 3, k = u % 3;
        if constexpr (k == 0) {
            constexpr bool single = 2 * tp + 1 >= 9;
            constexpr unsigned wimm = (unsigned)((6 * tp + 2) * 64) * 16u;
            static_assert(!single || wimm == W4_IMM, "tap 8");
            const unsigned wb = single ? x_w4 : x_w, sab = single ? x_sa4 : x_sa;
            const unsigned bb = tp == 0 ? hd_b : (single ? x_b4 : Lb + in_off + 2 * PLANE_S + tap_sel[tp] * 4u);
            const unsigned sbb = tp == 0 ? hd_sb : Lb + in_off + 3 * PLANE_S + tap_sel[tp];
_Pragma("unroll")
            for (int m = 0; m < 2; ++m) { f.a[m] = *(lds_cu32x4*)(at(wb) + wimm + m * 512); f.sa[m] = *(lds_cuchar*)(at(sab) + 128 * tp + m * 32); }
_Pragma("unroll")
            for (int q = 0; q < 2; ++q) {
                f.b[q] = *(lds_cu32x4*)(at(bb) + q * QS);
                f.sb[q] = *(lds_cint*)(at(sbb) + q * (QS >> 2));
            }
        } else {
            constexpr int tap = 2 * tp + k - 1;
            const unsigned pb = b_off + tap_s(tap / 3, tap % 3);
_Pragma("unroll")
            for (int m = 0; m < 2; ++m) f.a[m] = *(lds_cu32x4*)(at(a_off) + ((tap * WPL) * 64) * 16 + m * 512);
_Pragma("unroll")
            for (int q = 0; q < 2; ++q) f.b[q] = *(lds_cu32x4*)(at(pb) + q * QS);
        }
    };
    auto mma_unit = [&](auto u_c, Frag& f, auto first_c) __attribute__((always_inline)) {
        constexpr int u = decltype(u_c)::value, k = u % 3;
        constexpr bool FIRST = decltype(first_c)::value && u == 0;
_Pragma("unroll")
        for (int m = 0; m < 2; ++m)
_Pragma("unroll")
            for (int q = 0; q < 2; ++q) {
                if constexpr (k != 0) wsu_mfma_f16(f.a[m], f.b[q], acc[m][q]);
                else if constexpr (FIRST) acc[m][q] = wsu_mfma_q4_z(f.a[m], f.b[q], f.sa[m], f.sb[q]);
                else wsu_mfma_q4(f.a[m], f.b[q], f.sa[m], f.sb[q], acc[m][q]);
            }
    };
    auto skip_units = [&](auto first_c) __attribute__((always_inline)) {
        constexpr bool FIRST = decltype(first_c)::value;
        if constexpr (!H) {
            constexpr int NU = 14;
            Frag fr[2];
            load_unit(std::integral_constant<int, 0>{}, fr[0]);
            WSU_STATIC_FOR(NU, u, {
                if constexpr (u + 1 < NU) load_unit(std::integral_constant<int, u + 1>{}, fr[(u + 1) % 2]);
                __builtin_amdgcn_sched_barrier(0);
                mma_unit(u_c, fr[u % 2], first_c);
                __builtin_amdgcn_sched_barrier(0);
            });
        } else {
            WSU_STATIC_FOR(9, tap, {
                u32x4 ah[2], bh[2];
                const unsigned pb = b_off + tap_s(tap / 3, tap % 3);
_Pragma("unroll")
                for (int m = 0; m < 2; ++m) ah[m] = *(lds_cu32x4*)(at(a_off) + ((tap * WPL) * 64) * 16 + m * 512);
_Pragma("unroll")
                for (int q = 0; q < 2; ++q) bh[q] = *(lds_cu32x4*)(at(pb) + q * QS);
_Pragma("unroll")
                for (int m = 0; m < 2; ++m)
_Pragma("unroll")
                    for (int q = 0; q < 2; ++q) {
                        if constexpr (FIRST && tap == 0) acc[m][q] = wsu_mfma_f16_z(ah[m], bh[q]);
                        else wsu_mfma_f16(ah[m], bh[q], acc[m][q]);
                    }
            });
        }
    };
    auto low_units = [&](auto dy_c) __attribute__((always_inline)) {
        constexpr int dy = decltype(dy_c)::value;
        constexpr unsigned WDY = dy ? (unsigned)(OFF_LW1) : 0u;
        const unsigned rowo = (unsigned)(((py + dy) * LP + px) * 16);
        if constexpr (!H) {
            const int u = cls * 2 + hh_q;
            u32x4 a4[2], b4[2]; int sa[2], sb[2];
            const unsigned pb = rowo + (unsigned)hh_q * 16u + laneL;
            const unsigned wb = dy == 0 ? hd_w : Lb + w_off + WDY + (unsigned)((u * 3 + 2) * 64 + l31) * 16u;
            const unsigned sab = dy == 0 ? hd_sa : Lb + w_off + WDY + W_GRAN_L + (unsigned)(u * 64 + l31);
            const unsigned bb = dy == 0 ? hd_b : Lb + in_off + 2 * PLANE_L + pb;
            const unsigned sbb = dy == 0 ? hd_sb : Lb + in_off + 3 * PLANE_L + (pb >> 2);
_Pragma("unroll")
            for (int m = 0; m < 2; ++m) { a4[m] = *(lds_cu32x4*)(at(wb) + m * 512); sa[m] = *(lds_cuchar*)(at(sab) + m * 32); }
_Pragma("unroll")
            for (int q = 0; q < 2; ++q) {
                b4[q] = *(lds_cu32x4*)(at(bb) + q * QL);
                sb[q] = *(lds_cint*)(at(sbb) + q * (QL >> 2));
            }
_Pragma("unroll")
            for (int m = 0; m < 2; ++m)
_Pragma("unroll")
                for (int q = 0; q < 2; ++q) wsu_mfma_q4(a4[m], b4[q], sa[m], sb[q], acc[m][q]);
        }
        WSU_STATIC_FOR(2, dx, {
            u32x4 ah[2], bh[2];
            const unsigned wb = a_off + WDY + (unsigned)(((cls * 2 + dx) * WPL) * 64) * 16u;
            const unsigned pb = b_off + rowo + dx * 16u;
_Pragma("unroll")
            for (int m = 0; m < 2; ++m) ah[m] = *(lds_cu32x4*)(at(wb) + m * 512);
_Pragma("unroll")
            for (int q = 0; q < 2; ++q) bh[q] = *(lds_cu32x4*)(at(pb) + q * QL);
_Pragma("unroll")
            for (int m = 0; m < 2; ++m)
_Pragma("unroll")
                for (int q = 0; q < 2; ++q) wsu_mfma_f16(ah[m], bh[q], acc[m][q]);
        });
    };

    auto finish_tile = [&]() __attribute__((always_inline)) {
        int l31o = l31, hho = hh, lro = lrow, lco = lcol;
        asm volatile("" : "+v"(l31o), "+v"(hho), "+v"(lro), "+v"(lco));
        const unsigned hw16 = (unsigned)(a.h * a.w) * 16u;
        const unsigned cbytes = (unsigned)wsu_q_chunk_bytes(a.h, a.w);
        const int nco = a.cout >> 4;
        const int X = cur.x0 + 2 * lco + px;
        const int Y0 = cur.y0 + 2 * (4 * rh + lro) + py, Y1 = Y0 + 4;
        const bool ok0 = Y0 < a.h && X < a.w, ok1 = Y1 < a.h && X < a.w;
        const unsigned off0 = (unsigned)(Y0 * a.w + X) * 16u, off1 = (unsigned)(Y1 * a.w + X) * 16u;
        const unsigned so0 = wsu_q_soff(Y0, X, a.tiles_x), so1 = wsu_q_soff(Y1, X, a.tiles_x);
        const unsigned hpl = hho ? hw16 : 0u;
        const bool okm = hho ? ok1 : ok0;
        unsigned og0 = ok0 ? off0 + hpl : OOB, og1 = ok1 ? off1 + hpl : OOB;
        unsigned oq = okm ? (hho ? off1 : off0) + 2u * hw16 : OOB, os = okm ? 3u * hw16 + (hho ? so1 : so0) : OOB;
        asm volatile("" : "+v"(og0), "+v"(og1), "+v"(oq), "+v"(os));
        const float relu_floor = a.relu ? 0.f : -__builtin_inff();
        float vmax = 0.f;
        WSU_STATIC_FOR(2, m, {
            WSU_STATIC_FOR(2, cp, {
                const int oc = cur.cb * 4 + m * 2 + cp;
                const int co0 = oc * 16 + 4 * hho;
                const f32x4 bx = *reinterpret_cast<const f32x4*>(s_bias + co0), by = *reinterpret_cast<const f32x4*>(s_bias + co0 + 8);
                f32x4 vx[2], vy[2];
_Pragma("unroll")
                for (int q = 0; q < 2; ++q)
_Pragma("unroll")
                    for (int e = 0; e < 4; ++e) {
                        const float x = fmaxf(acc[m][q][8 * cp + e] + bx[e], relu_floor), y = fmaxf(acc[m][q][8 * cp + 4 + e] + by[e], relu_floor);
                        vx[q][e] = x; vy[q][e] = y;
                        if constexpr (H) vmax = fmaxf(fmaxf(vmax, fabsf(x)), fabsf(y));
                    }
                if constexpr (H) {
                    char* base = a.y + ((size_t)cur.n * nco + oc) * (2u * hw16);
                    const auto rs = __builtin_amdgcn_make_buffer_rsrc(base, 0, (int)(2u * hw16), 0x00020000);
                    __builtin_amdgcn_raw_buffer_store_b128(wsu_h_granule(vx[0], vy[0]), rs, (int)og0, 0, 0);
                    __builtin_amdgcn_raw_buffer_store_b128(wsu_h_granule(vx[1], vy[1]), rs, (int)og1, 0, 0);
                    return;
                }
                u32x4 g0, g1; uint32_t dh0, dr0, sb0, dh1, dr1, sb1;
                const float mx0 = wsu_q4_pre(vx[0], vy[0], g0, dh0, dr0, sb0);
                const float mx1 = wsu_q4_pre(vx[1], vy[1], g1, dh1, dr1, sb1);
                vmax = wsu_max3(vmax, mx0, mx1);
                const u32x4 qg = wsu_q4_pair(dh0, dr0, dh1, dr1);
                char* base = a.y + ((size_t)cur.n * nco + oc) * cbytes;
                const auto rs = __builtin_amdgcn_make_buffer_rsrc(base, 0, (int)cbytes, 0x00020000);
                __builtin_amdgcn_raw_buffer_store_b128(g0, rs, (int)og0, 0, 0);
                __builtin_amdgcn_raw_buffer_store_b128(g1, rs, (int)og1, 0, 0);
                __builtin_amdgcn_raw_buffer_store_b128(qg, rs, (int)oq, 0, 0);
                __builtin_amdgcn_raw_buffer_store_b8((unsigned char)(hho ? sb1 : sb0), rs, (int)os, 0, 0);
            });
        });
        if (a.range_flag && __builtin_amdgcn_ballot_w64(!(vmax <= (H ? WSU_F16_RANGE : WSU_F8_RANGE))) != 0 && lane == 0) atomicOr(a.range_flag, 1u);
    };

    for (int t = 0; t < K; ++t) {
        sync_step(std::false_type{});
        skip_units(std::true_type{});
        for (int c = 1; c < a.nchS; ++c) {
            sync_step(std::false_type{});
            skip_units(std::false_type{});
        }
        for (int c = 0; c < a.nchL; ++c) {
            sync_step(std::true_type{});
            low_units(std::integral_constant<int, 0>{});
            low_units(std::integral_constant<int, 1>{});
        }
        finish_tile();
        if (t + 1 < K) cur = tile_of(a, lw + (t + 1) * G);
    }
}

template <int FMT>
__global__ void pack_up_low_kernel(const float* __restrict__ w3, const float* __restrict__ wt, char* __restrict__ dst, float* __restrict__ wc_dense,
                                   int cup, int c2, int cl, int cout) {
    const int nchL = cl / 16, ctot = cup + c2;
    const long long total = (long long)(cout / WSU_COB) * nchL * 2 * W_UNITS_L * WSU_COB;
    for (long long d = (long long)blockIdx.x * blockDim.x + threadIdx.x; d < total; d += (long long)gridDim.x * blockDim.x) {
        long long t = d;
        const int co = (int)(t % WSU_COB); t /= WSU_COB;
        const int u = (int)(t % W_UNITS_L); t /= W_UNITS_L;
        const int dy = (int)(t & 1); t >>= 1;
        const int c = (int)(t % nchL); const int cb = (int)(t / nchL);
        const int cls = u >> 1, dx = u & 1, py = cls >> 1, px = cls & 1;
        const int ky0 = py == 0 ? (dy == 0 ? 0 : 1) : (dy == 0 ? 0 : 2), ky1 = py == 0 ? (dy == 0 ? 0 : 2) : (dy == 0 ? 1 : 2);
        const int kx0 = px == 0 ? (dx == 0 ? 0 : 1) : (dx == 0 ? 0 : 2), kx1 = px == 0 ? (dx == 0 ? 0 : 2) : (dx == 0 ? 1 : 2);
        const int cog = cb * WSU_COB + co;
        float v[16], r[16];
#pragma unroll
        for (int e = 0; e < 16; ++e) v[e] = 0.f;
        for (int ci = 0; ci < cup; ++ci)
            for (int ky = ky0; ky <= ky1; ++ky)
                for (int kx = kx0; kx <= kx1; ++kx) {
                    const float w = w3[(((size_t)cog * ctot + ci) * 3 + ky) * 3 + kx];
                    const int sy = (py + ky + 1) & 1, sx = (px + kx + 1) & 1;
#pragma unroll
                    for (int e = 0; e < 16; ++e) v[e] = fmaf(w, wt[(((size_t)(c * 16 + e) * cup + ci) * 2 + sy) * 2 + sx], v[e]);
                }
        if (wc_dense)
#pragma unroll
            for (int e = 0; e < 16; ++e) wc_dense[((((size_t)cog * cl + c * 16 + e) * 2 + py) * 2 + px) * 4 + dy * 2 + dx] = v[e];
        uint32_t h[8];
#pragma unroll
        for (int e = 0; e < 8; ++e) {
            const _Float16 x = (_Float16)v[2 * e], y = (_Float16)v[2 * e + 1];
            h[e] = (uint32_t)__builtin_bit_cast(unsigned short, x) | ((uint32_t)__builtin_bit_cast(unsigned short, y) << 16);
            r[2 * e] = (v[2 * e] - (float)x) * 2048.f; r[2 * e + 1] = (v[2 * e + 1] - (float)y) * 2048.f;
        }
        const u32x4 h0 = mk_u4(h[0], h[1], h[2], h[3]), h1 = mk_u4(h[4], h[5], h[6], h[7]);
        if constexpr (FMT == WSU_PLANAR_H) {
            char* base = dst + (((size_t)cb * nchL + c) * 2 + dy) * W_L_H + (size_t)(u * 2) * (WSU_COB * 16) + co * 16;
            *reinterpret_cast<u32x4*>(base) = h0;
            *reinterpret_cast<u32x4*>(base + WSU_COB * 16) = h1;
            continue;
        }
        const int E = wsu_q4_block_exp(wsu_f16x16_max_abs_bits(h0, h1));
        const float sc = wsu_pow2f(E);
        uint32_t q[4] = {0, 0, 0, 0};
        WSU_STATIC_FOR(8, e, { q[e >> 2] = __builtin_amdgcn_cvt_scalef32_pk_fp4_f32(q[e >> 2], r[2 * e], r[2 * e + 1], sc, e & 3); });
        q[2] = wsu_f16x8_to_fp4(h0, sc); q[3] = wsu_f16x8_to_fp4(h1, sc);
        char* slice = dst + (((size_t)cb * nchL + c) * 2 + dy) * W_L;
        char* base = slice + (size_t)(u * 3) * (WSU_COB * 16) + co * 16;
        *reinterpret_cast<u32x4*>(base) = h0;
        *reinterpret_cast<u32x4*>(base + WSU_COB * 16) = h1;
        *reinterpret_cast<u32x4*>(base + 2 * WSU_COB * 16) = mk_u4(q[0], q[1], q[2], q[3]);
        slice[W_GRAN_L + u * 64 + co] = (char)(E + 127 - 11);
        if (u == 0 && co < 32) *reinterpret_cast<u32x4*>(slice + W_GRAN_L + 512 + co * 16) = mk_u4(0, 0, 0, 0);
    }
}

__global__ void up_bias_kernel(const float* __restrict__ w3, const float* __restrict__ bt, const float* __restrict__ b3, float* __restrict__ out, int cup, int c2, int cout) {
    const int co = blockIdx.x * blockDim.x + threadIdx.x;
    if (co >= cout) return;
    float s = b3 ? b3[co] : 0.f;
    if (bt)
        for (int ci = 0; ci < cup; ++ci) {
            float t = 0.f;
            for (int k = 0; k < 9; ++k) t += w3[((size_t)co * (cup + c2) + ci) * 9 + k];
            s = fmaf(bt[ci], t, s);
        }
    out[co] = s;
}

struct UFormat {
    const char* pack; const char* fwd;
    void (*pack_kernel)(const float*, const float*, char*, float*, int, int, int, int); const char* pack_kernel_name;
    void (*kernel)(const UArgs); const char* kernel_name; const char* lds_name;
    int w_s, w_l;
};
const UFormat& u_format(int fmt) {
    static const UFormat q = {"conv3x3_up_pack", "conv3x3_up_q", pack_up_low_kernel<WSU_PLANAR_Q>, "pack_up_low_kernel",
                              conv3x3_qu_kernel<WSU_PLANAR_Q>, "conv3x3_qu_kernel", "conv3x3_qu", W_S, W_L};
    static const UFormat h = {"conv3x3_up_pack_h", "conv3x3_up_h", pack_up_low_kernel<WSU_PLANAR_H>, "pack_up_low_kernel<H>",
                              conv3x3_qu_kernel<WSU_PLANAR_H>, "conv3x3_qu_kernel<H>", "conv3x3_qu<H>", W_S_H, W_L_H};
    return fmt == WSU_PLANAR_H ? h : q;
}

size_t up_packed_bytes(int fmt, int cl, int cout) {
    if (cl <= 0 || cout <= 0 || cl % 16 || cout % WSU_COB) return 0;
    return (size_t)(cout / WSU_COB) * (cl / 16) * 2 * u_format(fmt).w_l;
}

int up_pack(int fmt, const float* w3_oihw, const float* wt, const float* bt, const float* b3, void* w_low_packed, float* bias_out, float* wc_dense,
            int cl, int cup, int c2, int cout, void* stream) {
    const UFormat& f = u_format(fmt);
    WSU_REQUIRE(w3_oihw && wt && w_low_packed && bias_out, "%s: null pointer", f.pack);
    WSU_REQUIRE(cl > 0 && cl % 16 == 0 && cup > 0 && c2 >= 0 && cout > 0 && cout % WSU_COB == 0,
                "%s: cl=%d must be a multiple of 16, cout=%d of %d, cup=%d > 0", f.pack, cl, cout, WSU_COB, cup);
    hipStream_t s = static_cast<hipStream_t>(stream);
    hipLaunchKernelGGL(f.pack_kernel, dim3(1024), dim3(128), 0, s, w3_oihw, wt, (char*)w_low_packed, wc_dense, cup, c2, cl, cout);
    int rc = wsu_check_launch(f.pack_kernel_name);
    if (rc != WSU_OK) return rc;
    hipLaunchKernelGGL(up_bias_kernel, dim3((cout + 63) / 64), dim3(64), 0, s, w3_oihw, bt, b3, bias_out, cup, c2, cout);
    return wsu_check_launch("up_bias_kernel");
}

int up_fwd(int fmt, const void* x_low, const void* x_skip, const void* w_skip_packed, const void* w_low_packed, const float* bias, void* y,
           int n, int h, int w, int cl, int c2, int cout, int relu, unsigned* range_flag, void* stream) {
    const UFormat& f = u_format(fmt);
    const char* who = f.fwd;
    WSU_REQUIRE(x_low && x_skip && w_skip_packed && w_low_packed && y, "%s: null pointer", who);
    WSU_REQUIRE(n > 0 && h >= 2 && w >= 2 && h % 2 == 0 && w % 2 == 0, "%s: bad shape n=%d h=%d w=%d (the output of a stride-2 transposed conv is even)", who, n, h, w);
    WSU_REQUIRE(cl > 0 && cl % 16 == 0 && c2 > 0 && c2 % 16 == 0, "%s: cl=%d c2=%d must be positive multiples of 16", who, cl, c2);
    WSU_REQUIRE(cout > 0 && cout % WSU_COB == 0 && cout <= MAX_COUT, "%s: cout=%d must be a multiple of %d (<= %d)", who, cout, WSU_COB, MAX_COUT);
    WSU_REQUIRE((long long)h * w * 50 < 0xFFFFFFF0LL, "%s: h*w too large (a chunk must stay below 4 GiB)", who);
    UArgs a;
    a.xl = (const char*)x_low; a.xs = (const char*)x_skip; a.wps = (const char*)w_skip_packed; a.wpl = (const char*)w_low_packed; a.bias = bias;
    a.y = (char*)y;
    a.n = n; a.h = h; a.w = w; a.hl = h / 2; a.wl = w / 2; a.cl = cl; a.c2 = c2; a.cout = cout;
    a.tiles_x = (w + TW - 1) / TW; a.tiles_y = (h + TH - 1) / TH; a.ltiles_x = (a.wl + 31) / 32; a.ncb = cout / WSU_COB;
    a.nchS = c2 / 16; a.nchL = cl / 16; a.relu = relu; a.range_flag = range_flag;
    const long long nt = (long long)n * a.tiles_x * a.tiles_y * a.ncb;
    WSU_REQUIRE(nt > 0 && nt < 0x3FFFFFFFLL, "%s: %lld tiles out of range", who, nt);
    WSU_REQUIRE((long long)a.ncb * a.nchL * 2 * f.w_l < 0x7FFFFFF0LL && (long long)a.ncb * a.nchS * f.w_s < 0x7FFFFFF0LL, "%s: packed weights beyond 2 GiB", who);
    a.ntiles = (int)nt;
    const int ncu = wsu_cu_count(who);
    if (!ncu) return WSU_ERR_HIP;
    static bool raised[2] = {false, false};
    bool& done = raised[fmt == WSU_PLANAR_H];
    if (!done) {
        if (int rc = wsu_raise_lds(f.kernel, LDS_TOTAL, f.lds_name)) return rc;
        done = true;
    }
    hipLaunchKernelGGL(f.kernel, dim3(a.ntiles < ncu ? a.ntiles : ncu), dim3(NT), LDS_TOTAL, static_cast<hipStream_t>(stream), a);
    return wsu_check_launch(f.kernel_name);
}

}

extern "C" {

size_t wsu_conv3x3_up_packed_bytes(int cl, int cout) { return up_packed_bytes(WSU_PLANAR_Q, cl, cout); }

int wsu_conv3x3_up_pack(const float* w3_oihw, const float* wt, const float* bt, const float* b3, void* w_low_packed, float* bias_out, float* wc_dense,
                        int cl, int cup, int c2, int cout, void* stream) {
    return up_pack(WSU_PLANAR_Q, w3_oihw, wt, bt, b3, w_low_packed, bias_out, wc_dense, cl, cup, c2, cout, stream);
}

int wsu_conv3x3_up_q_fwd(const void* x_low, const void* x_skip, const void* w_skip_packed, const void* w_low_packed, const float* bias, void* y,
                         int n, int h, int w, int cl, int c2, int cout, int relu, unsigned* range_flag, void* stream) {
    return up_fwd(WSU_PLANAR_Q, x_low, x_skip, w_skip_packed, w_low_packed, bias, y, n, h, w, cl, c2, cout, relu, range_flag, stream);
}

size_t wsu_conv3x3_up_packed_h_bytes(int cl, int cout) { return up_packed_bytes(WSU_PLANAR_H, cl, cout); }

int wsu_conv3x3_up_pack_h(const float* w3_oihw, const float* wt, const float* bt, const float* b3, void* w_low_packed, float* bias_out, float* wc_dense,
                          int cl, int cup, int c2, int cout, void* stream) {
    return up_pack(WSU_PLANAR_H, w3_oihw, wt, bt, b3, w_low_packed, bias_out, wc_dense, cl, cup, c2, cout, stream);
}

int wsu_conv3x3_up_h_fwd(const void* x_low, const void* x_skip, const void* w_skip_packed, const void* w_low_packed, const float* bias, void* y,
                         int n, int h, int w, int cl, int c2, int cout, int relu, unsigned* range_flag, void* stream) {
    return up_fwd(WSU_PLANAR_H, x_low, x_skip, w_skip_packed, w_low_packed, bias, y, n, h, w, cl, c2, cout, relu, range_flag, stream);
}

}
```

### ws_unet_amd/csrc/wsu_device.h

```cpp
#pragma once
#include <hip/hip_runtime.h>
#include <stdint.h>
#include <type_traits>
#include "../../include/wsu.h"

typedef __attribute__((ext_vector_type(8))) __bf16 bf16x8;
typedef __attribute__((ext_vector_type(16))) float f32x16;
typedef __attribute__((ext_vector_type(4))) float f32x4;
typedef __attribute__((ext_vector_type(4))) uint32_t u32x4;
typedef __attribute__((ext_vector_type(2))) uint32_t u32x2;
__host__ __device__ __forceinline__ u32x4 mk_u4(uint32_t a, uint32_t b, uint32_t c, uint32_t d) { u32x4 v = {a, b, c, d}; return v; }
__host__ __device__ __forceinline__ u32x2 mk_u2(uint32_t a, uint32_t b) { u32x2 v = {a, b}; return v; }
__host__ __device__ __forceinline__ f32x4 mk_f4(float a, float b, float c, float d) { f32x4 v = {a, b, c, d}; return v; }

void wsu_set_error(const char* fmt, ...);
int wsu_check_launch(const char* what);
#define WSU_REQUIRE(cond, ...)            \
    do {                                  \
        if (!(cond)) {                    \
            wsu_set_error(__VA_ARGS__);   \
            return WSU_ERR_ARG;           \
        }                                 \
    } while (0)
constexpr long long WSU_COUNTER_PIXELS = 1LL << 32;
constexpr long long WSU_PATH_PIXELS = 1LL << 31;
#define WSU_REQUIRE_SHAPE(what, limit, noun)                                                                           \
    WSU_REQUIRE(n > 0 && n <= 65535 && h >= 1 && w >= 1, what ": bad shape n=%d h=%d w=%d", n, h, w);                 \
    WSU_REQUIRE((long long)h * w < (limit), what ": %lld pixels per image exceed the 32-bit " noun, (long long)h * w)
#define WSU_REQUIRE_INTERIOR(who, cap_bits)                                                                            \
    WSU_REQUIRE(n > 0 && n <= 65535 && h >= 3 && w >= 3, "%s: bad shape n=%d h=%d w=%d", who, n, h, w);               \
    WSU_REQUIRE((cap_bits) <= 0 || (long long)(h - 2) * (w - 2) <= (1LL << (cap_bits)), "%s: %lld interior pixels per image exceed 2^%d", who, \
                (long long)(h - 2) * (w - 2), (int)(cap_bits))
#define WSU_INTERNAL extern "C" __attribute__((visibility("hidden")))
WSU_INTERNAL int wsu_cu_count(const char* who);
WSU_INTERNAL int wsu_raise_lds_ptr(const void* kernel, int bytes, const char* who);
template <class... A> inline int wsu_raise_lds(void (*kernel)(A...), int bytes, const char* who) {
    return wsu_raise_lds_ptr(reinterpret_cast<const void*>(kernel), bytes, who);
}
constexpr int WSU_LDS_DEFAULT = 64 * 1024;
constexpr int WSU_LDS_CU = 160 * 1024;

#define WSU_GRAN 4
#define WSU_COB 64
__host__ __device__ inline int wsu_chunk_channels(int mode) { return mode == WSU_MODE_BF16 ? 32 : 16; }

__device__ __forceinline__ int wsu_reflect(int i, int n) {
    i = i < 0 ? -i : i;
    i = i >= n ? 2 * (n - 1) - i : i;
    return min(max(i, 0), n - 1);
}

__device__ __forceinline__ uint32_t wsu_pack_bf16x2(float a, float b) {
    __bf16 x = (__bf16)a, y = (__bf16)b;
    return (uint32_t)__builtin_bit_cast(uint16_t, x) | ((uint32_t)__builtin_bit_cast(uint16_t, y) << 16);
}
__device__ __forceinline__ float wsu_bf16_lo_residual(float a) { return a - (float)(__bf16)a; }

__device__ __forceinline__ void wsu_split2(float a, float b, uint32_t& hi, uint32_t& lo) {
    const uint32_t ra = __builtin_bit_cast(uint32_t, a) + 0x8000u, rb = __builtin_bit_cast(uint32_t, b) + 0x8000u;
    hi = __builtin_amdgcn_perm(rb, ra, 0x07060302u);
    lo = wsu_pack_bf16x2(a - __builtin_bit_cast(float, ra & 0xFFFF0000u), b - __builtin_bit_cast(float, rb & 0xFFFF0000u));
}
__device__ __forceinline__ void wsu_split8(const f32x4& a, const f32x4& b, u32x4& hi, u32x4& lo) {
    uint32_t h0, h1, h2, h3, l0, l1, l2, l3;
    wsu_split2(a.x, a.y, h0, l0); wsu_split2(a.z, a.w, h1, l1);
    wsu_split2(b.x, b.y, h2, l2); wsu_split2(b.z, b.w, h3, l3);
    hi = mk_u4(h0, h1, h2, h3); lo = mk_u4(l0, l1, l2, l3);
}

typedef __attribute__((ext_vector_type(8))) _Float16 f16x8;
typedef __attribute__((ext_vector_type(8))) int i32x8;
#define WSU_F8_XLO_DIV 0x1p-12f
#define WSU_F8_X_DIV 4.f
#define WSU_F8_W_DIV 0x1p-6f
#define WSU_F8_WLO_DIV 0x1p-18f
#define WSU_F8_SCALE_XLO 115
#define WSU_F8_SCALE_X 129
#define WSU_F8_SCALE_W 121
#define WSU_F8_SCALE_WLO 109
#define WSU_F8_GLO_DIV 0x1p-14f
#define WSU_F8_G_DIV 0.25f
#define WSU_F8_SCALE_GLO 113
#define WSU_F8_SCALE_G 125
#define WSU_F8_RANGE 448.f
typedef __attribute__((ext_vector_type(2))) float f32x2;
typedef __attribute__((ext_vector_type(2))) _Float16 f16x2;
typedef __attribute__((ext_vector_type(2))) short i16x2;
__device__ __forceinline__ float wsu_sub_f16_lo(float v, uint32_t hpair) {
    float r; asm("v_fma_mix_f32 %0, %1, -1.0, %2 op_sel_hi:[1,0,0]" : "=v"(r) : "v"(hpair), "v"(v)); return r;
}
__device__ __forceinline__ float wsu_sub_f16_hi(float v, uint32_t hpair) {
    float r; asm("v_fma_mix_f32 %0, %1, -1.0, %2 op_sel:[1,0,0] op_sel_hi:[1,0,0]" : "=v"(r) : "v"(hpair), "v"(v)); return r;
}
__device__ __forceinline__ float wsu_fma_f16_lo(float a, float b, uint32_t hpair) {
    float r; asm("v_fma_mix_f32 %0, %1, %2, %3 op_sel_hi:[0,0,1]" : "=v"(r) : "v"(a), "v"(b), "v"(hpair)); return r;
}
__device__ __forceinline__ float wsu_fma_f16_hi(float a, float b, uint32_t hpair) {
    float r; asm("v_fma_mix_f32 %0, %1, %2, %3 op_sel:[0,0,1] op_sel_hi:[0,0,1]" : "=v"(r) : "v"(a), "v"(b), "v"(hpair)); return r;
}
__device__ __forceinline__ unsigned wsu_f16x8_pos_bits(const u32x4& h) {
    unsigned bits = 0;
#pragma unroll
    for (int e = 0; e < 4; ++e) {
        const int wd = (int)h[e];
        bits |= ((short)(wd & 0xFFFF) > 0 ? 1u : 0u) << (2 * e);
        bits |= (wd >= 0x10000 ? 1u : 0u) << (2 * e + 1);
    }
    return bits;
}
__host__ __device__ inline int wsu_mask_wp(int w) { return (w + 31) & ~31; }
__host__ __device__ inline int wsu_mask_hp(int h) { return (h + 15) & ~15; }
__device__ __forceinline__ float wsu_add_f16_lo(float acc, uint32_t hpair) {
    float r; asm("v_fma_mix_f32 %0, %1, 1.0, %2 op_sel_hi:[1,0,0]" : "=v"(r) : "v"(hpair), "v"(acc)); return r;
}
__device__ __forceinline__ float wsu_add_f16_hi(float acc, uint32_t hpair) {
    float r; asm("v_fma_mix_f32 %0, %1, 1.0, %2 op_sel:[1,0,0] op_sel_hi:[1,0,0]" : "=v"(r) : "v"(hpair), "v"(acc)); return r;
}
__device__ __forceinline__ void wsu_split4_f16f8(const f32x4& v, float div_lo, float div_x, uint32_t& h01, uint32_t& h23, uint32_t& lo, uint32_t& x8) {
    const f32x2 a = {v[0], v[1]}, b = {v[2], v[3]};
    const f16x2 ha = __builtin_convertvector(a, f16x2), hb = __builtin_convertvector(b, f16x2);
    h01 = __builtin_bit_cast(uint32_t, ha); h23 = __builtin_bit_cast(uint32_t, hb);
    const float lim_lo = 448.f * div_lo, lim_x = 448.f * div_x;
    const float r0 = __builtin_amdgcn_fmed3f(wsu_sub_f16_lo(v[0], h01), -lim_lo, lim_lo), r1 = __builtin_amdgcn_fmed3f(wsu_sub_f16_hi(v[1], h01), -lim_lo, lim_lo);
    const float r2 = __builtin_amdgcn_fmed3f(wsu_sub_f16_lo(v[2], h23), -lim_lo, lim_lo), r3 = __builtin_amdgcn_fmed3f(wsu_sub_f16_hi(v[3], h23), -lim_lo, lim_lo);
    i16x2 l = {0, 0}, x = {0, 0};
    l = __builtin_amdgcn_cvt_scalef32_pk_fp8_f32(l, r0, r1, div_lo, false);
    l = __builtin_amdgcn_cvt_scalef32_pk_fp8_f32(l, r2, r3, div_lo, true);
    x = __builtin_amdgcn_cvt_scalef32_pk_fp8_f32(x, __builtin_amdgcn_fmed3f(v[0], -lim_x, lim_x), __builtin_amdgcn_fmed3f(v[1], -lim_x, lim_x), div_x, false);
    x = __builtin_amdgcn_cvt_scalef32_pk_fp8_f32(x, __builtin_amdgcn_fmed3f(v[2], -lim_x, lim_x), __builtin_amdgcn_fmed3f(v[3], -lim_x, lim_x), div_x, true);
    lo = __builtin_bit_cast(uint32_t, l); x8 = __builtin_bit_cast(uint32_t, x);
}
__device__ __forceinline__ void wsu_split4_f16r8(const f32x4& v, float div_lo, uint32_t& h01, uint32_t& h23, uint32_t& lo) {
    const f32x2 a = {v[0], v[1]}, b = {v[2], v[3]};
    const f16x2 ha = __builtin_convertvector(a, f16x2), hb = __builtin_convertvector(b, f16x2);
    h01 = __builtin_bit_cast(uint32_t, ha); h23 = __builtin_bit_cast(uint32_t, hb);
    const float lim_lo = 448.f * div_lo;
    const float r0 = __builtin_amdgcn_fmed3f(wsu_sub_f16_lo(v[0], h01), -lim_lo, lim_lo), r1 = __builtin_amdgcn_fmed3f(wsu_sub_f16_hi(v[1], h01), -lim_lo, lim_lo);
    const float r2 = __builtin_amdgcn_fmed3f(wsu_sub_f16_lo(v[2], h23), -lim_lo, lim_lo), r3 = __builtin_amdgcn_fmed3f(wsu_sub_f16_hi(v[3], h23), -lim_lo, lim_lo);
    i16x2 l = {0, 0};
    l = __builtin_amdgcn_cvt_scalef32_pk_fp8_f32(l, r0, r1, div_lo, false);
    l = __builtin_amdgcn_cvt_scalef32_pk_fp8_f32(l, r2, r3, div_lo, true);
    lo = __builtin_bit_cast(uint32_t, l);
}
__device__ __forceinline__ void wsu_split16_f16f8(const f32x4& q0, const f32x4& q1, const f32x4& q2, const f32x4& q3,
                                                  u32x4& hi0, u32x4& hi1, u32x4& lo8) {
    uint32_t a0, a1, a2, a3, a4, a5, a6, a7, l0, l1, l2, l3, x0, x1, x2, x3;
    wsu_split4_f16f8(q0, WSU_F8_XLO_DIV, WSU_F8_X_DIV, a0, a1, l0, x0); wsu_split4_f16f8(q1, WSU_F8_XLO_DIV, WSU_F8_X_DIV, a2, a3, l1, x1);
    wsu_split4_f16f8(q2, WSU_F8_XLO_DIV, WSU_F8_X_DIV, a4, a5, l2, x2); wsu_split4_f16f8(q3, WSU_F8_XLO_DIV, WSU_F8_X_DIV, a6, a7, l3, x3);
    hi0 = mk_u4(a0, a1, a2, a3); hi1 = mk_u4(a4, a5, a6, a7); lo8 = mk_u4(l0, l1, l2, l3);
}
__device__ __forceinline__ u32x2 wsu_f16x8_to_fp8(const u32x4& h) {
    const _Float16 m = (_Float16)1792.f;
    const f16x8 lim = {m, m, m, m, m, m, m, m};
    const f16x8 c = __builtin_elementwise_max(__builtin_elementwise_min(__builtin_bit_cast(f16x8, h), lim), -lim);
    i16x2 lo = {0, 0}, hi = {0, 0};
    lo = __builtin_amdgcn_cvt_scalef32_pk_fp8_f16(lo, __builtin_shufflevector(c, c, 0, 1), WSU_F8_X_DIV, false);
    lo = __builtin_amdgcn_cvt_scalef32_pk_fp8_f16(lo, __builtin_shufflevector(c, c, 2, 3), WSU_F8_X_DIV, true);
    hi = __builtin_amdgcn_cvt_scalef32_pk_fp8_f16(hi, __builtin_shufflevector(c, c, 4, 5), WSU_F8_X_DIV, false);
    hi = __builtin_amdgcn_cvt_scalef32_pk_fp8_f16(hi, __builtin_shufflevector(c, c, 6, 7), WSU_F8_X_DIV, true);
    return mk_u2(__builtin_bit_cast(uint32_t, lo), __builtin_bit_cast(uint32_t, hi));
}
typedef __attribute__((ext_vector_type(2))) _Float16 f16x2_t;
typedef __attribute__((ext_vector_type(2))) unsigned short u16x2_t;
__device__ __forceinline__ int wsu_q4_block_exp(uint32_t b) {
    const int ef = (int)(b >> 10);
    return ef - 16 - ((ef > 0 && (b & 0x3FFu) <= 0x200u) ? 1 : 0);
}
__device__ __forceinline__ float wsu_pow2f(int e) { return __builtin_bit_cast(float, (uint32_t)(e + 127) << 23); }
__device__ __forceinline__ uint32_t wsu_f16x16_max_abs_bits(const u32x4& h0, const u32x4& h1) {
    u16x2_t m = __builtin_bit_cast(u16x2_t, h0.x & 0x7FFF7FFFu);
    m = __builtin_elementwise_max(m, __builtin_bit_cast(u16x2_t, h0.y & 0x7FFF7FFFu));
    m = __builtin_elementwise_max(m, __builtin_bit_cast(u16x2_t, h0.z & 0x7FFF7FFFu));
    m = __builtin_elementwise_max(m, __builtin_bit_cast(u16x2_t, h0.w & 0x7FFF7FFFu));
    m = __builtin_elementwise_max(m, __builtin_bit_cast(u16x2_t, h1.x & 0x7FFF7FFFu));
    m = __builtin_elementwise_max(m, __builtin_bit_cast(u16x2_t, h1.y & 0x7FFF7FFFu));
    m = __builtin_elementwise_max(m, __builtin_bit_cast(u16x2_t, h1.z & 0x7FFF7FFFu));
    m = __builtin_elementwise_max(m, __builtin_bit_cast(u16x2_t, h1.w & 0x7FFF7FFFu));
    return m.x > m.y ? m.x : m.y;
}
__device__ __forceinline__ uint32_t wsu_f16x8_to_fp4(const u32x4& h, float scale) {
    uint32_t d = 0;
    asm volatile("v_cvt_scalef32_pk_fp4_f16 %0, %1, %2" : "+v"(d) : "v"(h.x), "v"(scale));
    asm volatile("v_cvt_scalef32_pk_fp4_f16 %0, %1, %2 op_sel:[0,0,1,0]" : "+v"(d) : "v"(h.y), "v"(scale));
    asm volatile("v_cvt_scalef32_pk_fp4_f16 %0, %1, %2 op_sel:[0,0,0,1]" : "+v"(d) : "v"(h.z), "v"(scale));
    asm volatile("v_cvt_scalef32_pk_fp4_f16 %0, %1, %2 op_sel:[0,0,1,1]" : "+v"(d) : "v"(h.w), "v"(scale));
    return d;
}
__host__ __device__ inline size_t wsu_q_sblocks(int h, int w) { return (size_t)((h + 15) >> 4) * (size_t)((w + 31) >> 5); }
__host__ __device__ inline size_t wsu_q_chunk_bytes(int h, int w) { return (size_t)48 * h * w + 512 * wsu_q_sblocks(h, w); }
__device__ __forceinline__ unsigned wsu_q_soff(int y, int x, int tiles_x) {
    return (unsigned)(((y >> 4) * tiles_x + (x >> 5)) * 512 + (y & 15) * 32 + (x & 31));
}
__device__ __forceinline__ void wsu_swap32(uint32_t& upper_of, uint32_t& lower_of) {
    const auto r = __builtin_amdgcn_permlane32_swap(upper_of, lower_of, false, false);
    upper_of = r[0]; lower_of = r[1];
}
__device__ __forceinline__ void wsu_q4_pre_cvt(const f32x4& X, const f32x4& Y, uint32_t& xh0, uint32_t& xh1, uint32_t& yh0, uint32_t& yh1) {
    const f32x2 xa = {X[0], X[1]}, xb = {X[2], X[3]}, ya = {Y[0], Y[1]}, yb = {Y[2], Y[3]};
    xh0 = __builtin_bit_cast(uint32_t, __builtin_convertvector(xa, f16x2)); xh1 = __builtin_bit_cast(uint32_t, __builtin_convertvector(xb, f16x2));
    yh0 = __builtin_bit_cast(uint32_t, __builtin_convertvector(ya, f16x2)); yh1 = __builtin_bit_cast(uint32_t, __builtin_convertvector(yb, f16x2));
}
__device__ __forceinline__ void wsu_q4_pre_enc(const f32x4& X, const f32x4& Y, uint32_t xh0, uint32_t xh1, uint32_t yh0, uint32_t yh1, uint32_t mb,
                                               u32x4& g, uint32_t& dhi, uint32_t& dres, uint32_t& sb) {
    const float r0 = wsu_sub_f16_lo(X[0], xh0), r1 = wsu_sub_f16_hi(X[1], xh0), r2 = wsu_sub_f16_lo(X[2], xh1), r3 = wsu_sub_f16_hi(X[3], xh1);
    const float r4 = wsu_sub_f16_lo(Y[0], yh0), r5 = wsu_sub_f16_hi(Y[1], yh0), r6 = wsu_sub_f16_lo(Y[2], yh1), r7 = wsu_sub_f16_hi(Y[3], yh1);
    uint32_t mw = mb, mp = mb;
    wsu_swap32(mw, mp);
    const int e = wsu_q4_block_exp(mw > mp ? mw : mp);
    const float sc = wsu_pow2f(e), scr = wsu_pow2f(e - 11);
    sb = (uint32_t)(e + 127);
    uint32_t dh = 0, dr = 0;
    asm volatile("v_cvt_scalef32_pk_fp4_f16 %0, %1, %2" : "+v"(dh) : "v"(xh0), "v"(sc));
    asm volatile("v_cvt_scalef32_pk_fp4_f16 %0, %1, %2 op_sel:[0,0,1,0]" : "+v"(dh) : "v"(xh1), "v"(sc));
    asm volatile("v_cvt_scalef32_pk_fp4_f16 %0, %1, %2 op_sel:[0,0,0,1]" : "+v"(dh) : "v"(yh0), "v"(sc));
    asm volatile("v_cvt_scalef32_pk_fp4_f16 %0, %1, %2 op_sel:[0,0,1,1]" : "+v"(dh) : "v"(yh1), "v"(sc));
    dr = __builtin_amdgcn_cvt_scalef32_pk_fp4_f32(dr, r0, r1, scr, 0);
    dr = __builtin_amdgcn_cvt_scalef32_pk_fp4_f32(dr, r2, r3, scr, 1);
    dr = __builtin_amdgcn_cvt_scalef32_pk_fp4_f32(dr, r4, r5, scr, 2);
    dr = __builtin_amdgcn_cvt_scalef32_pk_fp4_f32(dr, r6, r7, scr, 3);
    dhi = dh; dres = dr;
    wsu_swap32(xh0, yh0); wsu_swap32(xh1, yh1);
    g = mk_u4(xh0, xh1, yh0, yh1);
}
__device__ __forceinline__ float wsu_q4_pre(const f32x4& X, const f32x4& Y, u32x4& g, uint32_t& dhi, uint32_t& dres, uint32_t& sb) {
    uint32_t xh0, xh1, yh0, yh1;
    wsu_q4_pre_cvt(X, Y, xh0, xh1, yh0, yh1);
    float mx = __builtin_fmaxf(__builtin_fmaxf(__builtin_fabsf(X[0]), __builtin_fabsf(X[1])), __builtin_fabsf(X[2]));
    mx = __builtin_fmaxf(__builtin_fmaxf(mx, __builtin_fabsf(X[3])), __builtin_fabsf(Y[0]));
    mx = __builtin_fmaxf(__builtin_fmaxf(mx, __builtin_fabsf(Y[1])), __builtin_fabsf(Y[2]));
    mx = __builtin_fmaxf(mx, __builtin_fabsf(Y[3]));
    const f32x2 mm = {mx, 0.f};
    wsu_q4_pre_enc(X, Y, xh0, xh1, yh0, yh1, __builtin_bit_cast(uint32_t, __builtin_convertvector(mm, f16x2)), g, dhi, dres, sb);
    return mx;
}
__device__ __forceinline__ void wsu_q4_pre_bits(const f32x4& X, const f32x4& Y, u32x4& g, uint32_t& dhi, uint32_t& dres, uint32_t& sb) {
    uint32_t xh0, xh1, yh0, yh1;
    wsu_q4_pre_cvt(X, Y, xh0, xh1, yh0, yh1);
    u16x2_t m = __builtin_elementwise_max(__builtin_bit_cast(u16x2_t, xh0 & 0x7FFF7FFFu), __builtin_bit_cast(u16x2_t, xh1 & 0x7FFF7FFFu));
    m = __builtin_elementwise_max(m, __builtin_bit_cast(u16x2_t, yh0 & 0x7FFF7FFFu));
    m = __builtin_elementwise_max(m, __builtin_bit_cast(u16x2_t, yh1 & 0x7FFF7FFFu));
    wsu_q4_pre_enc(X, Y, xh0, xh1, yh0, yh1, m.x > m.y ? m.x : m.y, g, dhi, dres, sb);
}
__device__ __forceinline__ float wsu_max3(float a, float b, float c) {
    float r; asm volatile("v_max3_f32 %0, %1, %2, %3" : "=v"(r) : "v"(a), "v"(b), "v"(c)); return r;
}
__device__ __forceinline__ u32x4 wsu_q4_pair(uint32_t dhi0, uint32_t dres0, uint32_t dhi1, uint32_t dres1) {
    wsu_swap32(dhi0, dhi1); wsu_swap32(dres0, dres1);
    return mk_u4(__builtin_amdgcn_perm(dhi1, dhi0, 0x05040100u), __builtin_amdgcn_perm(dhi1, dhi0, 0x07060302u),
                 __builtin_amdgcn_perm(dres1, dres0, 0x05040100u), __builtin_amdgcn_perm(dres1, dres0, 0x07060302u));
}
__device__ __forceinline__ u32x4 wsu_q4_single(uint32_t dhi, uint32_t dres) {
    uint32_t ph = dhi, pr = dres;
    wsu_swap32(dhi, ph); wsu_swap32(dres, pr);
    return mk_u4(__builtin_amdgcn_perm(ph, dhi, 0x05040100u), __builtin_amdgcn_perm(ph, dhi, 0x07060302u),
                 __builtin_amdgcn_perm(pr, dres, 0x05040100u), __builtin_amdgcn_perm(pr, dres, 0x07060302u));
}
#define WSU_F16_RANGE 65504.f
__host__ __device__ inline size_t wsu_h_chunk_bytes(int h, int w) { return (size_t)32 * h * w; }
__device__ __forceinline__ u32x4 wsu_h_granule(const f32x4& X, const f32x4& Y) {
    const f32x2 xa = {X[0], X[1]}, xb = {X[2], X[3]}, ya = {Y[0], Y[1]}, yb = {Y[2], Y[3]};
    uint32_t xh0 = __builtin_bit_cast(uint32_t, __builtin_convertvector(xa, f16x2)), xh1 = __builtin_bit_cast(uint32_t, __builtin_convertvector(xb, f16x2));
    uint32_t yh0 = __builtin_bit_cast(uint32_t, __builtin_convertvector(ya, f16x2)), yh1 = __builtin_bit_cast(uint32_t, __builtin_convertvector(yb, f16x2));
    wsu_swap32(xh0, yh0); wsu_swap32(xh1, yh1);
    return mk_u4(xh0, xh1, yh0, yh1);
}
__device__ __forceinline__ void wsu_q4_encode16(const f32x4 (&v)[4], u32x4& h0, u32x4& h1, u32x4& q, uint32_t& sb) {
    uint32_t h[8]; float r[16];
#pragma unroll
    for (int k = 0; k < 4; ++k) {
        const f32x2 a = {v[k][0], v[k][1]}, b = {v[k][2], v[k][3]};
        h[2 * k] = __builtin_bit_cast(uint32_t, __builtin_convertvector(a, f16x2)); h[2 * k + 1] = __builtin_bit_cast(uint32_t, __builtin_convertvector(b, f16x2));
        r[4 * k] = wsu_sub_f16_lo(v[k][0], h[2 * k]); r[4 * k + 1] = wsu_sub_f16_hi(v[k][1], h[2 * k]);
        r[4 * k + 2] = wsu_sub_f16_lo(v[k][2], h[2 * k + 1]); r[4 * k + 3] = wsu_sub_f16_hi(v[k][3], h[2 * k + 1]);
    }
    h0 = mk_u4(h[0], h[1], h[2], h[3]); h1 = mk_u4(h[4], h[5], h[6], h[7]);
    const int e = wsu_q4_block_exp(wsu_f16x16_max_abs_bits(h0, h1));
    const float sc = wsu_pow2f(e), scr = wsu_pow2f(e - 11);
    sb = (uint32_t)(e + 127);
    uint32_t q2 = 0, q3 = 0;
    q2 = __builtin_amdgcn_cvt_scalef32_pk_fp4_f32(q2, r[0], r[1], scr, 0); q2 = __builtin_amdgcn_cvt_scalef32_pk_fp4_f32(q2, r[2], r[3], scr, 1);
    q2 = __builtin_amdgcn_cvt_scalef32_pk_fp4_f32(q2, r[4], r[5], scr, 2); q2 = __builtin_amdgcn_cvt_scalef32_pk_fp4_f32(q2, r[6], r[7], scr, 3);
    q3 = __builtin_amdgcn_cvt_scalef32_pk_fp4_f32(q3, r[8], r[9], scr, 0); q3 = __builtin_amdgcn_cvt_scalef32_pk_fp4_f32(q3, r[10], r[11], scr, 1);
    q3 = __builtin_amdgcn_cvt_scalef32_pk_fp4_f32(q3, r[12], r[13], scr, 2); q3 = __builtin_amdgcn_cvt_scalef32_pk_fp4_f32(q3, r[14], r[15], scr, 3);
    q = mk_u4(wsu_f16x8_to_fp4(h0, sc), wsu_f16x8_to_fp4(h1, sc), q2, q3);
}
__device__ __forceinline__ void wsu_mfma_q4(const u32x4& a, const u32x4& b, int scale_a, int scale_b, f32x16& acc) {
    const i32x8 av = {(int)a.x, (int)a.y, (int)a.z, (int)a.w, 0, 0, 0, 0}, bv = {(int)b.x, (int)b.y, (int)b.z, (int)b.w, 0, 0, 0, 0};
    acc = __builtin_amdgcn_mfma_scale_f32_32x32x64_f8f6f4(av, bv, acc, 4, 4, 0, scale_a, 0, scale_b);
}

__device__ __forceinline__ f32x16 wsu_mfma_q4_z(const u32x4& a, const u32x4& b, int scale_a, int scale_b) {
    const i32x8 av = {(int)a.x, (int)a.y, (int)a.z, (int)a.w, 0, 0, 0, 0}, bv = {(int)b.x, (int)b.y, (int)b.z, (int)b.w, 0, 0, 0, 0};
    const f32x16 z = {0.f, 0.f, 0.f, 0.f, 0.f, 0.f, 0.f, 0.f, 0.f, 0.f, 0.f, 0.f, 0.f, 0.f, 0.f, 0.f};
    return __builtin_amdgcn_mfma_scale_f32_32x32x64_f8f6f4(av, bv, z, 4, 4, 0, scale_a, 0, scale_b);
}

__device__ __forceinline__ u32x2 wsu_f16x8_to_fp8_grad(const u32x4& h) {
    const _Float16 m = (_Float16)112.f;
    const f16x8 lim = {m, m, m, m, m, m, m, m};
    const f16x8 c = __builtin_elementwise_max(__builtin_elementwise_min(__builtin_bit_cast(f16x8, h), lim), -lim);
    i16x2 lo = {0, 0}, hi = {0, 0};
    lo = __builtin_amdgcn_cvt_scalef32_pk_fp8_f16(lo, __builtin_shufflevector(c, c, 0, 1), WSU_F8_G_DIV, false);
    lo = __builtin_amdgcn_cvt_scalef32_pk_fp8_f16(lo, __builtin_shufflevector(c, c, 2, 3), WSU_F8_G_DIV, true);
    hi = __builtin_amdgcn_cvt_scalef32_pk_fp8_f16(hi, __builtin_shufflevector(c, c, 4, 5), WSU_F8_G_DIV, false);
    hi = __builtin_amdgcn_cvt_scalef32_pk_fp8_f16(hi, __builtin_shufflevector(c, c, 6, 7), WSU_F8_G_DIV, true);
    return mk_u2(__builtin_bit_cast(uint32_t, lo), __builtin_bit_cast(uint32_t, hi));
}
__device__ __forceinline__ void wsu_mfma_f16(const u32x4& a, const u32x4& b, f32x16& acc) {
    acc = __builtin_amdgcn_mfma_f32_32x32x16_f16(__builtin_bit_cast(f16x8, a), __builtin_bit_cast(f16x8, b), acc, 0, 0, 0);
}
__device__ __forceinline__ f32x16 wsu_mfma_f16_z(const u32x4& a, const u32x4& b) {
    const f32x16 z = {0.f, 0.f, 0.f, 0.f, 0.f, 0.f, 0.f, 0.f, 0.f, 0.f, 0.f, 0.f, 0.f, 0.f, 0.f, 0.f};
    return __builtin_amdgcn_mfma_f32_32x32x16_f16(__builtin_bit_cast(f16x8, a), __builtin_bit_cast(f16x8, b), z, 0, 0, 0);
}
__device__ __forceinline__ void wsu_mfma_f8x2(const u32x4& a_blk0, const u32x4& a_blk1, const u32x4& b_blk0, const u32x4& b_blk1,
                                              int scale_a, int scale_b, f32x16& acc) {
    i32x8 a = {(int)a_blk0.x, (int)a_blk0.y, (int)a_blk0.z, (int)a_blk0.w, (int)a_blk1.x, (int)a_blk1.y, (int)a_blk1.z, (int)a_blk1.w};
    i32x8 b = {(int)b_blk0.x, (int)b_blk0.y, (int)b_blk0.z, (int)b_blk0.w, (int)b_blk1.x, (int)b_blk1.y, (int)b_blk1.z, (int)b_blk1.w};
    acc = __builtin_amdgcn_mfma_scale_f32_32x32x64_f8f6f4(a, b, acc, 0, 0, 0, scale_a, 0, scale_b);
}

__device__ __forceinline__ float wsu_bf16_to_f32(uint16_t v) { return __builtin_bit_cast(float, (uint32_t)v << 16); }

template <int MODE>
__device__ __forceinline__ void wsu_mfma_step(const u32x4& a, const u32x4& b, f32x16& acc) {
    if constexpr (MODE == WSU_MODE_F32) {
        const f32x4 af = __builtin_bit_cast(f32x4, a), bf = __builtin_bit_cast(f32x4, b);
        acc = __builtin_amdgcn_mfma_f32_32x32x2f32(af[0], bf[0], acc, 0, 0, 0);
        acc = __builtin_amdgcn_mfma_f32_32x32x2f32(af[1], bf[1], acc, 0, 0, 0);
        acc = __builtin_amdgcn_mfma_f32_32x32x2f32(af[2], bf[2], acc, 0, 0, 0);
        acc = __builtin_amdgcn_mfma_f32_32x32x2f32(af[3], bf[3], acc, 0, 0, 0);
    } else {
        acc = __builtin_amdgcn_mfma_f32_32x32x16_bf16(__builtin_bit_cast(bf16x8, a), __builtin_bit_cast(bf16x8, b), acc, 0, 0, 0);
    }
}

template <int N> struct wsu_static_for_t {
    template <class F> __device__ __forceinline__ static void run(F&& f) {
        wsu_static_for_t<N - 1>::run(f);
        f(std::integral_constant<int, N - 1>{});
    }
};
template <> struct wsu_static_for_t<0> { template <class F> __device__ __forceinline__ static void run(F&&) {} };
#define WSU_STATIC_FOR(N, VAR, ...) wsu_static_for_t<N>::run([&](auto VAR##_c) __attribute__((always_inline)) { constexpr int VAR = decltype(VAR##_c)::value; __VA_ARGS__ })

__device__ __forceinline__ unsigned wsu_xcd_remap(unsigned bid, unsigned nwg) {
    const unsigned q = nwg >> 3, r = nwg & 7u, xcd = bid & 7u, k = bid >> 3;
    const unsigned base = xcd < r ? xcd * (q + 1) : r * (q + 1) + (xcd - r) * q;
    return base + k;
}
```

Before: 3850.

## Store 16 channels per lane per row in conv epilogue with new channel-row map

Restructures the conv3x3 epilogue so each lane encodes and stores 16 channels of one row at a time (f16 halves plus fp4 residual and scale), rather than pairing two rows with cross-lane swaps. It adds a row-to-channel permutation helper and a BIG format variant that splits stores across two buffer descriptors when the output chunk exceeds 32-bit offsets. The aim is to cut per-element permute and swap work and to simplify the store addressing, at the cost of a changed weight/accumulator channel mapping that must stay consistent with the packers.

Measured after the change: 3879 (median of 6 runs). Within noise of the previous version (+0.8%).

```diff
diff --git a/ws_unet_amd/csrc/conv3x3_q.hip b/ws_unet_amd/csrc/conv3x3_q.hip
--- a/ws_unet_amd/csrc/conv3x3_q.hip
+++ b/ws_unet_amd/csrc/conv3x3_q.hip
@@ -20,6 +20,7 @@
 constexpr int NLOAD = 4;
 constexpr int W_PIECES = W_SLOT / 1024;
 constexpr unsigned OOB = 0xFFFFFFF0u;
+constexpr int FMT_BIG = 16;
 constexpr int IN_SLOT_H = 2 * PLANE;
 constexpr int W_SLOT_H = 9 * 2 * WSU_COB * 16;
 template <int FMT> struct QGeo {
@@ -232,9 +233,11 @@
     if (a.range_flag && __builtin_amdgcn_ballot_w64(!(f1_max <= WSU_F8_RANGE)) != 0 && lane == 0) atomicOr(a.range_flag, 1u);
 }
 
-template <int RQ, int HC, bool POOL, bool FQ, bool MSPLIT, bool F1 = false, int FMT = WSU_PLANAR_Q>
+template <int RQ, int HC, bool POOL, bool FQ, bool MSPLIT, bool F1 = false, int FMTB = WSU_PLANAR_Q>
 __global__ __launch_bounds__((16 / RQ + NLOAD) * 64) __attribute__((amdgpu_waves_per_eu(RQ == 4 ? 2 : 3, RQ == 4 ? 2 : 3)))
 void conv3x3_q_kernel(const QArgs a) {
+    constexpr int FMT = FMTB & ~FMT_BIG;
+    constexpr bool BIG = (FMTB & FMT_BIG) != 0;
     using Gm = QGeo<FMT>;
     constexpr bool H = Gm::H;
     static_assert(!(H && F1), "the fused first layer computes Q inputs");
@@ -457,176 +460,147 @@
         for (int q = 0; q < RQ; ++q)
 #pragma unroll
             for (int o = 0; o < (HC > 0 ? HC : 1); ++o) hz[q][o] = 0.f;
-        struct QOff { unsigned g0, g1, q, s; };
-        auto pair_off = [&](unsigned plane_bytes, unsigned off0, unsigned off1, unsigned soff0, unsigned soff1, bool ok0, bool ok1) __attribute__((always_inline)) {
-            const unsigned hp = hh ? plane_bytes : 0u;
-            const bool okm = hh ? ok1 : ok0;
-            QOff o = {ok0 ? off0 + hp : OOB, ok1 ? off1 + hp : OOB, okm ? (hh ? off1 : off0) + 2u * plane_bytes : OOB, okm ? 3u * plane_bytes + (hh ? soff1 : soff0) : OOB};
-            asm volatile("" : "+v"(o.g0), "+v"(o.g1), "+v"(o.q), "+v"(o.s));
+        constexpr bool YQ = FQ && !H;
+        struct LOff { unsigned g0, g1, q, s; };
+        auto lane_off = [&](unsigned plane_bytes, unsigned chunk, unsigned off, unsigned soff, bool ok, bool split) __attribute__((always_inline)) {
+            const unsigned ct = (hh && !split) ? chunk : 0u;
+            LOff o = {ok ? off + ct : OOB, ok ? off + plane_bytes + ct : OOB, OOB, OOB};
+            if constexpr (!H) o.q = ok ? off + 2u * plane_bytes + ct : OOB;
+            if constexpr (YQ) o.s = ok ? 3u * plane_bytes + soff + ct : OOB;
+            if constexpr (H) asm volatile("" : "+v"(o.g0), "+v"(o.g1));
+            else if constexpr (YQ) asm volatile("" : "+v"(o.g0), "+v"(o.g1), "+v"(o.q), "+v"(o.s));
+            else asm volatile("" : "+v"(o.g0), "+v"(o.g1), "+v"(o.q));
             return o;
         };
-        constexpr bool YQ = FQ && !H;
-        QOff qo[RQ / 2] = {}, qop = {};
-        if constexpr (YQ) {
+        const unsigned ychunk = H ? 2u * hw16 : (YQ ? (unsigned)wsu_q_chunk_bytes(a.h, a.w) : 3u * hw16);
+        LOff yo[RQ] = {}, po[RQ / 2] = {};
+        unsigned pchunk = 0;
+        {
             const unsigned sblk = (unsigned)(((cur.y0 >> 4) * a.tiles_x + (cur.x0 >> 5)) * 512);
 _Pragma("unroll")
-            for (int rp = 0; rp < RQ / 2; ++rp) {
-                const int r0 = RQ * wv + 2 * rp, row0 = cur.y0 + r0;
-                qo[rp] = pair_off(hw16, (unsigned)(row0 * a.w + col) * 16u, (unsigned)((row0 + 1) * a.w + col) * 16u,
-                                  sblk + (unsigned)(r0 * 32 + l31), sblk + (unsigned)((r0 + 1) * 32 + l31), row0 < a.h && col < a.w, row0 + 1 < a.h && col < a.w);
+            for (int q = 0; q < RQ; ++q) {
+                const int r = RQ * wv + q, row = cur.y0 + r;
+                yo[q] = lane_off(hw16, ychunk, (unsigned)(row * a.w + col) * 16u, sblk + (unsigned)(r * 32 + l31), row < a.h && col < a.w, BIG);
             }
             if constexpr (POOL) {
                 const int hp = a.h >> 1, wp2 = a.w >> 1, ptx = (wp2 + 31) >> 5;
                 const int gy0 = (cur.y0 >> 1) + (RQ / 2) * wv, gx = (cur.x0 >> 1) + (l31 >> 1);
                 const unsigned php16 = (unsigned)(hp * wp2) * 16u;
-                if constexpr (RQ == 4) {
-                    const bool okx = !(l31 & 1) && gx < wp2;
-                    qop = pair_off(php16, (unsigned)(gy0 * wp2 + gx) * 16u, (unsigned)((gy0 + 1) * wp2 + gx) * 16u,
-                                   wsu_q_soff(gy0, gx, ptx), wsu_q_soff(gy0 + 1, gx, ptx), okx && gy0 < hp, okx && gy0 + 1 < hp);
+                pchunk = H ? 2u * php16 : (YQ ? (unsigned)wsu_q_chunk_bytes(hp, wp2) : 3u * php16);
+                const bool okx = !(l31 & 1) && gx < wp2;
+_Pragma("unroll")
+                for (int rp = 0; rp < RQ / 2; ++rp)
+                    po[rp] = lane_off(php16, pchunk, (unsigned)((gy0 + rp) * wp2 + gx) * 16u, wsu_q_soff(gy0 + rp, gx, ptx), okx && gy0 + rp < hp, false);
+            }
+        }
+        auto store16 = [&](const f32x4 (&v)[4], char* base, unsigned chunk, const LOff& o, bool have, auto split_c) __attribute__((always_inline)) {
+            constexpr bool SPLIT = decltype(split_c)::value;
+            const auto rs0 = __builtin_amdgcn_make_buffer_rsrc(base, 0, have ? (int)(SPLIT ? chunk : 2u * chunk) : 0, 0x00020000);
+            const auto rs1 = __builtin_amdgcn_make_buffer_rsrc(base + (SPLIT ? chunk : 0u), 0, have ? (int)chunk : 0, 0x00020000);
+            auto st128 = [&](const u32x4& g, unsigned off) __attribute__((always_inline)) {
+                if constexpr (!SPLIT) {
+                    __builtin_amdgcn_raw_buffer_store_b128(g, rs0, (int)off, 0, 0);
                 } else {
-                    const unsigned coff = (l31 & 1) ? (unsigned)wsu_q_chunk_bytes(hp, wp2) : 0u;
-                    const unsigned off = (unsigned)(gy0 * wp2 + gx) * 16u + coff, soff = wsu_q_soff(gy0, gx, ptx) + coff;
-                    const bool ok = gx < wp2 && gy0 < hp;
-                    qop = {ok ? off + (hh ? php16 : 0u) : OOB, OOB, (ok && !hh) ? off + 2u * php16 : OOB, (ok && !hh) ? 3u * php16 + soff : OOB};
-                    asm volatile("" : "+v"(qop.g0), "+v"(qop.q), "+v"(qop.s));
+                    __builtin_amdgcn_raw_buffer_store_b128(g, rs0, (int)(hh ? OOB : off), 0, 0);
+                    __builtin_amdgcn_raw_buffer_store_b128(g, rs1, (int)(hh ? off : OOB), 0, 0);
                 }
-            }
-        }
-        auto store_pair_q = [&](const f32x4& X0, const f32x4& Y0, const f32x4& X1, const f32x4& Y1, char* base, unsigned chunk_bytes, const QOff& o, bool have, bool fold) __attribute__((always_inline)) {
-            u32x4 g0, g1; uint32_t dh0, dr0, sb0, dh1, dr1, sb1;
-            const float mx0 = wsu_q4_pre(X0, Y0, g0, dh0, dr0, sb0);
-            const float mx1 = wsu_q4_pre(X1, Y1, g1, dh1, dr1, sb1);
-            if (fold) vmax = wsu_max3(vmax, mx0, mx1);
-            const u32x4 qg = wsu_q4_pair(dh0, dr0, dh1, dr1);
-            const auto rs = __builtin_amdgcn_make_buffer_rsrc(base, 0, have ? (int)chunk_bytes : 0, 0x00020000);
-            __builtin_amdgcn_raw_buffer_store_b128(g0, rs, (int)o.g0, 0, 0);
-            __builtin_amdgcn_raw_buffer_store_b128(g1, rs, (int)o.g1, 0, 0);
-            __builtin_amdgcn_raw_buffer_store_b128(qg, rs, (int)o.q, 0, 0);
-            __builtin_amdgcn_raw_buffer_store_b8((unsigned char)(hh ? sb1 : sb0), rs, (int)o.s, 0, 0);
-        };
-        auto store_one_q = [&](const f32x4& X, const f32x4& Y, char* base, unsigned chunk_bytes, const QOff& o) __attribute__((always_inline)) {
-            u32x4 g; uint32_t dh, dr, sb;
-            wsu_q4_pre(X, Y, g, dh, dr, sb);
-            const u32x4 qg = wsu_q4_single(dh, dr);
-            const auto rs = __builtin_amdgcn_make_buffer_rsrc(base, 0, (int)chunk_bytes, 0x00020000);
-            __builtin_amdgcn_raw_buffer_store_b128(g, rs, (int)o.g0, 0, 0);
-            __builtin_amdgcn_raw_buffer_store_b128(qg, rs, (int)o.q, 0, 0);
-            __builtin_amdgcn_raw_buffer_store_b8((unsigned char)sb, rs, (int)o.s, 0, 0);
-        };
-        auto store_one_h = [&](const f32x4& X, const f32x4& Y, char* base, unsigned plane_bytes, unsigned off, bool ok, bool have) __attribute__((always_inline)) {
-            const auto rs = __builtin_amdgcn_make_buffer_rsrc(base, 0, have ? (int)(2u * plane_bytes) : 0, 0x00020000);
-            __builtin_amdgcn_raw_buffer_store_b128(wsu_h_granule(X, Y), rs, (int)(ok ? off + (hh ? plane_bytes : 0u) : OOB), 0, 0);
-        };
-        auto store_one_a = [&](const f32x4& X, const f32x4& Y, char* base, unsigned plane_bytes, unsigned off, bool ok, bool have) __attribute__((always_inline)) {
-            uint32_t xh0, xh1, xlo, yh0, yh1, ylo;
-            wsu_split4_f16r8(X, WSU_F8_XLO_DIV, xh0, xh1, xlo);
-            wsu_split4_f16r8(Y, WSU_F8_XLO_DIV, yh0, yh1, ylo);
-            wsu_swap32(xh0, yh0); wsu_swap32(xh1, yh1);
-            uint32_t xlp = xlo, ylp = ylo;
-            wsu_swap32(xlo, xlp); wsu_swap32(ylo, ylp);
-            const auto rs = __builtin_amdgcn_make_buffer_rsrc(base, 0, have ? (int)(3u * plane_bytes) : 0, 0x00020000);
-            __builtin_amdgcn_raw_buffer_store_b128(mk_u4(xh0, xh1, yh0, yh1), rs, (int)(ok ? off + (hh ? plane_bytes : 0u) : OOB), 0, 0);
-            __builtin_amdgcn_raw_buffer_store_b128(mk_u4(xlo, xlp, ylo, ylp), rs, (int)((ok && !hh) ? off + 2u * plane_bytes : OOB), 0, 0);
+            };
+            float mx = 0.f;
+            u32x4 h0, h1;
+            if constexpr (H) {
+                wsu_h_encode16(v, h0, h1);
+                st128(h0, o.g0); st128(h1, o.g1);
+            } else if constexpr (FQ) {
+                u32x4 qg; uint32_t sb;
+                mx = wsu_q4_encode16_max(v, h0, h1, qg, sb);
+                st128(h0, o.g0); st128(h1, o.g1); st128(qg, o.q);
+                if constexpr (!SPLIT) {
+                    __builtin_amdgcn_raw_buffer_store_b8((unsigned char)sb, rs0, (int)o.s, 0, 0);
+                } else {
+                    __builtin_amdgcn_raw_buffer_store_b8((unsigned char)sb, rs0, (int)(hh ? OOB : o.s), 0, 0);
+                    __builtin_amdgcn_raw_buffer_store_b8((unsigned char)sb, rs1, (int)(hh ? o.s : OOB), 0, 0);
+                }
+            } else {
+                u32x4 lo;
+                wsu_a_encode16(v, h0, h1, lo);
+                st128(h0, o.g0); st128(h1, o.g1); st128(lo, o.q);
+            }
+            return mx;
         };
         auto epi_m = [&](auto m_c, auto&& hook) __attribute__((always_inline)) {
             constexpr int m = decltype(m_c)::value;
-            constexpr int NH = RQ / 2;
-            f32x4 spx, spy;
-            auto piece = [&](auto cp_c) __attribute__((always_inline)) {
-                constexpr int cp = decltype(cp_c)::value;
-                const int oc = cur.cb * 4 + (m + cur.mh) * 2 + cp;
-                const int co0 = oc * 16 + 4 * hh;
-                const bool have_y = a.y != nullptr;
-                f32x4 px[2], py[2];
-                WSU_STATIC_FOR(RQ / 2, rp, {
-                    hook(std::integral_constant<int, NH * cp + rp>{});
-                    f32x4 vx[2], vy[2];
-                    const f32x4 bx = *reinterpret_cast<const f32x4*>(s_bias + co0), by = *reinterpret_cast<const f32x4*>(s_bias + co0 + 8);
-_Pragma("unroll")
-                    for (int u = 0; u < 2; ++u) {
-_Pragma("unroll")
-                        for (int e = 0; e < 4; ++e) {
-                            const float x = fmaxf(acc[m][2 * rp + u][8 * cp + e] + bx[e], relu_floor), y = fmaxf(acc[m][2 * rp + u][8 * cp + 4 + e] + by[e], relu_floor);
-                            vx[u][e] = x; vy[u][e] = y;
-                            if constexpr (H || !FQ) vmax = fmaxf(fmaxf(vmax, fabsf(x)), fabsf(y));
-                        }
+            const int oc0 = cur.cb * 4 + (m + cur.mh) * 2;
+            const bool have_y = a.y != nullptr;
+            f32x4 b[4];
+_Pragma("unroll")
+            for (int k = 0; k < 4; ++k) b[k] = *reinterpret_cast<const f32x4*>(s_bias + (oc0 + hh) * 16 + 4 * k);
+            f32x4 pv[4];
+            float mxe = 0.f;
+            WSU_STATIC_FOR(RQ, q, {
+                hook(q_c);
+                f32x4 v[4];
+_Pragma("unroll")
+                for (int k = 0; k < 4; ++k) {
+_Pragma("unroll")
+                    for (int e = 0; e < 4; ++e) v[k][e] = fmaxf(acc[m][q][4 * k + e] + b[k][e], relu_floor);
+                    if constexpr (H || !FQ) {
+                        vmax = fmaxf(fmaxf(vmax, fabsf(v[k][0])), fabsf(v[k][1]));
+                        vmax = fmaxf(fmaxf(vmax, fabsf(v[k][2])), fabsf(v[k][3]));
                     }
-                    if constexpr (HEAD) {
+                }
+                if (!HEAD || have_y) {
+                    char* base = a.y + ((size_t)cur.n * nco + oc0) * ychunk;
+                    const float mx = store16(v, base, ychunk, yo[q], have_y, std::integral_constant<bool, BIG>{});
+                    if constexpr (YQ) {
+                        if constexpr (q & 1) vmax = wsu_max3(vmax, mxe, mx);
+                        else mxe = mx;
+                    }
+                }
+                if constexpr (POOL) {
+                    if constexpr ((q & 1) == 0) {
+_Pragma("unroll")
+                        for (int k = 0; k < 4; ++k) pv[k] = v[k];
+                    } else {
+                        f32x4 pw[4];
+_Pragma("unroll")
+                        for (int k = 0; k < 4; ++k)
+_Pragma("unroll")
+                            for (int e = 0; e < 4; ++e) {
+                                const float c = fmaxf(pv[k][e], v[k][e]);
+                                pw[k][e] = fmaxf(c, dpp_xor1(c));
+                            }
+                        char* pbase = a.ypool + ((size_t)cur.n * nco + oc0) * pchunk;
+                        store16(pw, pbase, pchunk, po[q / 2], true, std::false_type{});
+                    }
+                }
+                if constexpr (HEAD) {
+_Pragma("unroll")
+                    for (int e = 0; e < 4; ++e) {
+                        const float f0 = v[0][e], f1 = v[1][e], f2 = v[2][e], f3 = v[3][e];
+                        uint32_t q0 = __builtin_bit_cast(uint32_t, f0), q1 = __builtin_bit_cast(uint32_t, f1);
+                        uint32_t q2 = __builtin_bit_cast(uint32_t, f2), q3 = __builtin_bit_cast(uint32_t, f3);
+                        wsu_swap32(q0, q1); wsu_swap32(q2, q3);
+                        v[0][e] = __builtin_bit_cast(float, q0); v[1][e] = __builtin_bit_cast(float, q1);
+                        v[2][e] = __builtin_bit_cast(float, q2); v[3][e] = __builtin_bit_cast(float, q3);
+                    }
+_Pragma("unroll")
+                    for (int cp = 0; cp < 2; ++cp) {
                         const int lc = (m * 2 + cp) * 16 + 4 * hh;
 _Pragma("unroll")
                         for (int o = 0; o < HC; ++o)
                             if (HC == 1 || o < a.head_cout)
 _Pragma("unroll")
-                                for (int u = 0; u < 2; ++u)
-_Pragma("unroll")
-                                    for (int e = 0; e < 4; ++e)
-                                        hz[2 * rp + u][o] = fmaf(vx[u][e], s_hw[o * 64 + lc + e], fmaf(vy[u][e], s_hw[o * 64 + lc + 8 + e], hz[2 * rp + u][o]));
+                                for (int e = 0; e < 4; ++e)
+                                    hz[q][o] = fmaf(v[cp][e], s_hw[o * 64 + lc + e], fmaf(v[2 + cp][e], s_hw[o * 64 + lc + 8 + e], hz[q][o]));
                     }
-                    const int r0 = RQ * wv + 2 * rp, row0 = cur.y0 + r0;
-                    if (!HEAD || have_y) {
-                        if constexpr (H) {
-                            char* base = a.y + ((size_t)cur.n * nco + oc) * (2u * hw16);
-                            WSU_STATIC_FOR(2, u, {
-                                store_one_h(vx[u], vy[u], base, hw16, (unsigned)((row0 + u) * a.w + col) * 16u, row0 + u < a.h && col < a.w, have_y);
-                            });
-                        } else if constexpr (FQ) {
-                            const unsigned cb_ = (unsigned)wsu_q_chunk_bytes(a.h, a.w);
-                            char* base = a.y + ((size_t)cur.n * nco + oc) * cb_;
-                            store_pair_q(vx[0], vy[0], vx[1], vy[1], base, cb_, qo[rp], have_y, true);
-                        } else {
-                            char* base = a.y + (((size_t)cur.n * nco + oc) * 3) * hw16;
-                            WSU_STATIC_FOR(2, u, {
-                                store_one_a(vx[u], vy[u], base, hw16, (unsigned)((row0 + u) * a.w + col) * 16u, row0 + u < a.h && col < a.w, have_y);
-                            });
-                        }
-                    }
-                    if constexpr (POOL) {
-_Pragma("unroll")
-                        for (int e = 0; e < 4; ++e) {
-                            const float cx = fmaxf(vx[0][e], vx[1][e]), cy = fmaxf(vy[0][e], vy[1][e]);
-                            px[rp][e] = fmaxf(cx, dpp_xor1(cx)); py[rp][e] = fmaxf(cy, dpp_xor1(cy));
-                        }
-                    }
-                });
-                if constexpr (POOL) {
-                    const int hp = a.h >> 1, wp2 = a.w >> 1;
-                    const int gy0 = (cur.y0 >> 1) + (RQ / 2) * wv, gx = (cur.x0 >> 1) + (l31 >> 1);
-                    const bool okx = !(l31 & 1) && gx < wp2;
-                    const unsigned php16 = (unsigned)(hp * wp2) * 16u;
-                    if constexpr (H) {
-                        char* base = a.ypool + ((size_t)cur.n * nco + oc) * (2u * php16);
-#pragma unroll
-                        for (int rp = 0; rp < RQ / 2; ++rp)
-                            store_one_h(px[rp], py[rp], base, php16, (unsigned)((gy0 + rp) * wp2 + gx) * 16u, okx && gy0 + rp < hp, true);
-                    } else if constexpr (FQ) {
-                        const unsigned cbp = (unsigned)wsu_q_chunk_bytes(hp, wp2);
-                        char* base = a.ypool + ((size_t)cur.n * nco + oc) * cbp;
-                        if constexpr (RQ == 4) {
-                            store_pair_q(px[0], py[0], px[1], py[1], base, cbp, qop, true, false);
-                        } else if constexpr (cp == 0) {
-                            spx = px[0]; spy = py[0];
-                        } else {
-                            static_assert(cp == 1, "piece 1 closes the pair: its chunk follows piece 0's");
-                            const bool odd = (l31 & 1) != 0;
-                            f32x4 sx, sy;
-_Pragma("unroll")
-                            for (int e = 0; e < 4; ++e) { sx[e] = odd ? px[0][e] : spx[e]; sy[e] = odd ? py[0][e] : spy[e]; }
-                            store_one_q(sx, sy, base - cbp, 2u * cbp, qop);
-                        }
-                    } else {
-                        char* base = a.ypool + (((size_t)cur.n * nco + oc) * 3) * php16;
-#pragma unroll
-                        for (int rp = 0; rp < RQ / 2; ++rp)
-                            store_one_a(px[rp], py[rp], base, php16, (unsigned)((gy0 + rp) * wp2 + gx) * 16u, okx && gy0 + rp < hp, true);
-                    }
+_Pragma("unroll")
+                    for (int o = 0; o < HC; ++o) asm volatile("" : "+v"(hz[q][o]));
                 }
-            };
-            piece(std::integral_constant<int, 0>{});
-            piece(std::integral_constant<int, 1>{});
+            });
         };
         auto nothing = [](auto) __attribute__((always_inline)) {};
         if constexpr (EPO) {
-            constexpr int NHT = 2 * (RQ / 2);
+            constexpr int NHT = RQ;
             epi_m(std::integral_constant<int, 0>{}, [&](auto h_c) __attribute__((always_inline)) {
                 constexpr int h = decltype(h_c)::value;
                 constexpr int lo = 5 * h / NHT, hi = 5 * (h + 1) / NHT;
@@ -685,10 +659,11 @@
         const int co = (int)(t % WSU_COB); t /= WSU_COB;
         const int tap = (int)(t % 9); t /= 9;
         const int c = (int)(t % nch); const int cb = (int)(t / nch);
+        const int ch = wsu_slot_channel(co);
         float v[16], r[16];
         uint32_t h[8];
 #pragma unroll
-        for (int e = 0; e < 16; ++e) v[e] = w[(((size_t)(cb * WSU_COB + co) * cin + c * 16 + e) * 3 + tap / 3) * 3 + tap % 3];
+        for (int e = 0; e < 16; ++e) v[e] = w[(((size_t)(cb * WSU_COB + ch) * cin + c * 16 + e) * 3 + tap / 3) * 3 + tap % 3];
 #pragma unroll
         for (int e = 0; e < 8; ++e) {
             const _Float16 a = (_Float16)v[2 * e], b = (_Float16)v[2 * e + 1];
@@ -720,10 +695,11 @@
         const int co = (int)(t % WSU_COB); t /= WSU_COB;
         const int tap = (int)(t % 9); t /= 9;
         const int c = (int)(t % nch); const int cb = (int)(t / nch);
+        const int ch = wsu_slot_channel(co);
         uint32_t h[8];
 #pragma unroll
         for (int e = 0; e < 8; ++e) {
-            const size_t i0 = (((size_t)(cb * WSU_COB + co) * cin + c * 16 + 2 * e) * 3 + tap / 3) * 3 + tap % 3;
+            const size_t i0 = (((size_t)(cb * WSU_COB + ch) * cin + c * 16 + 2 * e) * 3 + tap / 3) * 3 + tap % 3;
             const _Float16 a = (_Float16)w[i0], b = (_Float16)w[i0 + 9];
             h[e] = (uint32_t)__builtin_bit_cast(unsigned short, a) | ((uint32_t)__builtin_bit_cast(unsigned short, b) << 16);
         }
@@ -751,27 +727,45 @@
     X(2, 1, false, true, false, false, WSU_PLANAR_H) \
     X(2, 4, false, true, false, false, WSU_PLANAR_H) \
     X(2, 0, false, true, true, false, WSU_PLANAR_H)
+#define WSU_Q_VARIANTS_BIG(Y)                 \
+    Y(2, 0, false, false, false, WSU_PLANAR_Q) \
+    Y(2, 0, false, true, false, WSU_PLANAR_Q)  \
+    Y(2, 0, true, false, false, WSU_PLANAR_Q)  \
+    Y(2, 0, true, true, false, WSU_PLANAR_Q)   \
+    Y(2, 1, false, false, false, WSU_PLANAR_Q) \
+    Y(2, 4, false, false, false, WSU_PLANAR_Q) \
+    Y(2, 0, true, true, true, WSU_PLANAR_Q)    \
+    Y(2, 0, false, true, false, WSU_PLANAR_H)  \
+    Y(2, 0, true, true, false, WSU_PLANAR_H)   \
+    Y(2, 1, false, true, false, WSU_PLANAR_H)  \
+    Y(2, 4, false, true, false, WSU_PLANAR_H)
 #define WSU_Q_INST(RQ, HC, POOL, FQ, MSPLIT, F1, FMT) template __global__ void conv3x3_q_kernel<RQ, HC, POOL, FQ, MSPLIT, F1, FMT>(const QArgs);
+#define WSU_Q_INST_BIG(RQ, HC, POOL, FQ, F1, FMT) template __global__ void conv3x3_q_kernel<RQ, HC, POOL, FQ, false, F1, FMT | FMT_BIG>(const QArgs);
 WSU_Q_VARIANTS(WSU_Q_INST)
+WSU_Q_VARIANTS_BIG(WSU_Q_INST_BIG)
 
 struct QVariant {
-    int rq, hc; bool pool, fq, msplit, f1; int fmt;
+    int rq, hc; bool pool, fq, msplit, f1; int fmt; bool big;
     void (*kernel)(const QArgs);
     bool raised;
 };
-#define WSU_Q_ROW(RQ, HC, POOL, FQ, MSPLIT, F1, FMT) {RQ, HC, POOL, FQ, MSPLIT, F1, FMT, conv3x3_q_kernel<RQ, HC, POOL, FQ, MSPLIT, F1, FMT>, false},
-QVariant q_variants[] = {WSU_Q_VARIANTS(WSU_Q_ROW)};
+#define WSU_Q_ROW(RQ, HC, POOL, FQ, MSPLIT, F1, FMT) {RQ, HC, POOL, FQ, MSPLIT, F1, FMT, false, conv3x3_q_kernel<RQ, HC, POOL, FQ, MSPLIT, F1, FMT>, false},
+#define WSU_Q_ROW_BIG(RQ, HC, POOL, FQ, F1, FMT) {RQ, HC, POOL, FQ, false, F1, FMT, true, conv3x3_q_kernel<RQ, HC, POOL, FQ, false, F1, FMT | FMT_BIG>, false},
+QVariant q_variants[] = {WSU_Q_VARIANTS(WSU_Q_ROW) WSU_Q_VARIANTS_BIG(WSU_Q_ROW_BIG)};
 
 int q_launch(QArgs a, const char* who, int fmt, int rq, bool yq, bool msplit_on, hipStream_t s) {
     const bool h = fmt == WSU_PLANAR_H, f1 = a.img != nullptr;
+    const size_t ychunk = h ? wsu_h_chunk_bytes(a.h, a.w) : (yq && !a.head_w ? wsu_q_chunk_bytes(a.h, a.w) : (size_t)48 * a.h * a.w);
+    const bool big = a.y != nullptr && 2 * ychunk > 0xFFFFFFF0ull;
+    if (big) rq = 2;
     const int ncu = wsu_cu_count(who);
     if (!ncu) return WSU_ERR_HIP;
     const int hc = !a.head_w ? 0 : (a.head_cout == 1 ? 1 : 4);
     const bool pool = a.ypool != nullptr, fq = h || (yq && !hc);
-    a.msplit = !f1 && msplit_on && !hc && !pool && 2 * (long long)a.ntiles <= ncu;
+    a.msplit = !f1 && !big && msplit_on && !hc && !pool && 2 * (long long)a.ntiles <= ncu;
     if (a.msplit) { a.ncb *= 2; a.ntiles *= 2; }
     for (QVariant& v : q_variants) {
-        if (v.rq != rq || v.hc != hc || v.pool != pool || v.fq != fq || v.msplit != (a.msplit != 0) || v.f1 != f1 || v.fmt != fmt) continue;
+        if (v.rq != rq || v.hc != hc || v.pool != pool || v.fq != fq || v.msplit != (a.msplit != 0) || v.f1 != f1 || v.fmt != fmt || v.big != big) continue;
         const int lds = h ? QGeo<WSU_PLANAR_H>::lds_total : LDS_TOTAL;
         if (!v.raised) {
             if (int rc = wsu_raise_lds(v.kernel, lds, f1 ? "conv3x3_q<F1>" : (h ? "conv3x3_q<H>" : "conv3x3_q"))) return rc;
diff --git a/ws_unet_amd/csrc/conv3x3_qu.hip b/ws_unet_amd/csrc/conv3x3_qu.hip
--- a/ws_unet_amd/csrc/conv3x3_qu.hip
+++ b/ws_unet_amd/csrc/conv3x3_qu.hip
@@ -31,6 +31,7 @@
 static_assert(IN_S + W_S <= REGION - ZERO_BYTES && OFF_LW1 + W_L <= REGION - ZERO_BYTES && LDS_ZERO % 16 == 0 && ZERO_BYTES >= 2 * CW * 16 + 16 + 16, "zero block");
 constexpr int NLOAD = 4, NWAVE = 8, NT = (NWAVE + NLOAD) * 64;
 constexpr unsigned OOB = 0xFFFFFFF0u;
+constexpr int FMT_BIG = 16;
 constexpr int W_S_H = 9 * 2 * WSU_COB * 16;
 constexpr int W_L_H = W_UNITS_L * 2 * WSU_COB * 16;
 constexpr int PIECES_S_H = W_S_H / 1024, PIECES_L_H = W_L_H / 1024;
@@ -70,9 +71,9 @@
 }
 
 
-template <int FMT, int LW>
+template <int FMTB, int LW>
 __device__ __forceinline__ void u_loader(const UArgs& a, char* smem, int lane, int lw, int G, int K) {
-    constexpr bool H = FMT == WSU_PLANAR_H;
+    constexpr bool H = (FMTB & ~FMT_BIG) == WSU_PLANAR_H;
     constexpr int NSS = LW < 2 ? 3 : 2;
     constexpr int NSL = LW < 2 ? 2 : 1;
     constexpr int OPS_INS = (H ? 2 : 4) * NSS, OPS_INL = (H ? 2 : 4) * NSL;
@@ -197,9 +198,11 @@
     }
 }
 
-template <int FMT>
+template <int FMTB>
 __global__ __launch_bounds__(NT) __attribute__((amdgpu_waves_per_eu(3, 3)))
 void conv3x3_qu_kernel(const UArgs a) {
+    constexpr int FMT = FMTB & ~FMT_BIG;
+    constexpr bool BIG = (FMTB & FMT_BIG) != 0;
     constexpr bool H = FMT == WSU_PLANAR_H;
     constexpr int WPL = H ? 2 : 3;
     extern __shared__ __attribute__((aligned(16))) char smem[];
@@ -217,10 +220,10 @@
 
     if (wv >= NWAVE) {
         switch (wv - NWAVE) {
-            case 0: u_loader<FMT, 0>(a, smem, lane, lw, G, K); break;
-            case 1: u_loader<FMT, 1>(a, smem, lane, lw, G, K); break;
-            case 2: u_loader<FMT, 2>(a, smem, lane, lw, G, K); break;
-            default: u_loader<FMT, 3>(a, smem, lane, lw, G, K); break;
+            case 0: u_loader<FMTB, 0>(a, smem, lane, lw, G, K); break;
+            case 1: u_loader<FMTB, 1>(a, smem, lane, lw, G, K); break;
+            case 2: u_loader<FMTB, 2>(a, smem, lane, lw, G, K); break;
+            default: u_loader<FMTB, 3>(a, smem, lane, lw, G, K); break;
         }
         return;
     }
@@ -407,45 +410,62 @@
         const bool ok0 = Y0 < a.h && X < a.w, ok1 = Y1 < a.h && X < a.w;
         const unsigned off0 = (unsigned)(Y0 * a.w + X) * 16u, off1 = (unsigned)(Y1 * a.w + X) * 16u;
         const unsigned so0 = wsu_q_soff(Y0, X, a.tiles_x), so1 = wsu_q_soff(Y1, X, a.tiles_x);
-        const unsigned hpl = hho ? hw16 : 0u;
-        const bool okm = hho ? ok1 : ok0;
-        unsigned og0 = ok0 ? off0 + hpl : OOB, og1 = ok1 ? off1 + hpl : OOB;
-        unsigned oq = okm ? (hho ? off1 : off0) + 2u * hw16 : OOB, os = okm ? 3u * hw16 + (hho ? so1 : so0) : OOB;
-        asm volatile("" : "+v"(og0), "+v"(og1), "+v"(oq), "+v"(os));
+        const unsigned chunk = H ? 2u * hw16 : cbytes;
+        const unsigned ct = (hho && !BIG) ? chunk : 0u;
+        unsigned og0[2] = {ok0 ? off0 + ct : OOB, ok1 ? off1 + ct : OOB}, og1[2] = {ok0 ? off0 + hw16 + ct : OOB, ok1 ? off1 + hw16 + ct : OOB};
+        unsigned oq[2] = {OOB, OOB}, os[2] = {OOB, OOB};
+        if constexpr (!H) {
+            oq[0] = ok0 ? off0 + 2u * hw16 + ct : OOB; oq[1] = ok1 ? off1 + 2u * hw16 + ct : OOB;
+            os[0] = ok0 ? 3u * hw16 + so0 + ct : OOB; os[1] = ok1 ? 3u * hw16 + so1 + ct : OOB;
+            asm volatile("" : "+v"(oq[0]), "+v"(oq[1]), "+v"(os[0]), "+v"(os[1]));
+        }
+        asm volatile("" : "+v"(og0[0]), "+v"(og0[1]), "+v"(og1[0]), "+v"(og1[1]));
         const float relu_floor = a.relu ? 0.f : -__builtin_inff();
         float vmax = 0.f;
         WSU_STATIC_FOR(2, m, {
-            WSU_STATIC_FOR(2, cp, {
-                const int oc = cur.cb * 4 + m * 2 + cp;
-                const int co0 = oc * 16 + 4 * hho;
-                const f32x4 bx = *reinterpret_cast<const f32x4*>(s_bias + co0), by = *reinterpret_cast<const f32x4*>(s_bias + co0 + 8);
-                f32x4 vx[2], vy[2];
-_Pragma("unroll")
-                for (int q = 0; q < 2; ++q)
-_Pragma("unroll")
-                    for (int e = 0; e < 4; ++e) {
-                        const float x = fmaxf(acc[m][q][8 * cp + e] + bx[e], relu_floor), y = fmaxf(acc[m][q][8 * cp + 4 + e] + by[e], relu_floor);
-                        vx[q][e] = x; vy[q][e] = y;
-                        if constexpr (H) vmax = fmaxf(fmaxf(vmax, fabsf(x)), fabsf(y));
+            const int oc0 = cur.cb * 4 + m * 2;
+            f32x4 b[4];
+_Pragma("unroll")
+            for (int k = 0; k < 4; ++k) b[k] = *reinterpret_cast<const f32x4*>(s_bias + (oc0 + hho) * 16 + 4 * k);
+            char* base = a.y + ((size_t)cur.n * nco + oc0) * chunk;
+            const auto rs0 = __builtin_amdgcn_make_buffer_rsrc(base, 0, (int)(BIG ? chunk : 2u * chunk), 0x00020000);
+            const auto rs1 = __builtin_amdgcn_make_buffer_rsrc(base + (BIG ? chunk : 0u), 0, (int)chunk, 0x00020000);
+            auto st128 = [&](const u32x4& g, unsigned off) __attribute__((always_inline)) {
+                if constexpr (!BIG) {
+                    __builtin_amdgcn_raw_buffer_store_b128(g, rs0, (int)off, 0, 0);
+                } else {
+                    __builtin_amdgcn_raw_buffer_store_b128(g, rs0, (int)(hho ? OOB : off), 0, 0);
+                    __builtin_amdgcn_raw_buffer_store_b128(g, rs1, (int)(hho ? off : OOB), 0, 0);
+                }
+            };
+            float mx0 = 0.f;
+            WSU_STATIC_FOR(2, q, {
+                f32x4 v[4];
+_Pragma("unroll")
+                for (int k = 0; k < 4; ++k) {
+_Pragma("unroll")
+                    for (int e = 0; e < 4; ++e) v[k][e] = fmaxf(acc[m][q][4 * k + e] + b[k][e], relu_floor);
+                    if constexpr (H) {
+                        vmax = fmaxf(fmaxf(vmax, fabsf(v[k][0])), fabsf(v[k][1]));
+                        vmax = fmaxf(fmaxf(vmax, fabsf(v[k][2])), fabsf(v[k][3]));
                     }
+                }
+                u32x4 h0, h1;
                 if constexpr (H) {
-                    char* base = a.y + ((size_t)cur.n * nco + oc) * (2u * hw16);
-                    const auto rs = __builtin_amdgcn_make_buffer_rsrc(base, 0, (int)(2u * hw16), 0x00020000);
-                    __builtin_amdgcn_raw_buffer_store_b128(wsu_h_granule(vx[0], vy[0]), rs, (int)og0, 0, 0);
-                    __builtin_amdgcn_raw_buffer_store_b128(wsu_h_granule(vx[1], vy[1]), rs, (int)og1, 0, 0);
-                    return;
+                    wsu_h_encode16(v, h0, h1);
+                    st128(h0, og0[q]); st128(h1, og1[q]);
+                } else {
+                    u32x4 qg; uint32_t sb;
+                    const float mx = wsu_q4_encode16_max(v, h0, h1, qg, sb);
+                    if constexpr (q == 0) mx0 = mx; else vmax = wsu_max3(vmax, mx0, mx);
+                    st128(h0, og0[q]); st128(h1, og1[q]); st128(qg, oq[q]);
+                    if constexpr (!BIG) {
+                        __builtin_amdgcn_raw_buffer_store_b8((unsigned char)sb, rs0, (int)os[q], 0, 0);
+                    } else {
+                        __builtin_amdgcn_raw_buffer_store_b8((unsigned char)sb, rs0, (int)(hho ? OOB : os[q]), 0, 0);
+                        __builtin_amdgcn_raw_buffer_store_b8((unsigned char)sb, rs1, (int)(hho ? os[q] : OOB), 0, 0);
+                    }
                 }
-                u32x4 g0, g1; uint32_t dh0, dr0, sb0, dh1, dr1, sb1;
-                const float mx0 = wsu_q4_pre(vx[0], vy[0], g0, dh0, dr0, sb0);
-                const float mx1 = wsu_q4_pre(vx[1], vy[1], g1, dh1, dr1, sb1);
-                vmax = wsu_max3(vmax, mx0, mx1);
-                const u32x4 qg = wsu_q4_pair(dh0, dr0, dh1, dr1);
-                char* base = a.y + ((size_t)cur.n * nco + oc) * cbytes;
-                const auto rs = __builtin_amdgcn_make_buffer_rsrc(base, 0, (int)cbytes, 0x00020000);
-                __builtin_amdgcn_raw_buffer_store_b128(g0, rs, (int)og0, 0, 0);
-                __builtin_amdgcn_raw_buffer_store_b128(g1, rs, (int)og1, 0, 0);
-                __builtin_amdgcn_raw_buffer_store_b128(qg, rs, (int)oq, 0, 0);
-                __builtin_amdgcn_raw_buffer_store_b8((unsigned char)(hho ? sb1 : sb0), rs, (int)os, 0, 0);
             });
         });
         if (a.range_flag && __builtin_amdgcn_ballot_w64(!(vmax <= (H ? WSU_F16_RANGE : WSU_F8_RANGE))) != 0 && lane == 0) atomicOr(a.range_flag, 1u);
@@ -482,7 +502,7 @@
         const int cls = u >> 1, dx = u & 1, py = cls >> 1, px = cls & 1;
         const int ky0 = py == 0 ? (dy == 0 ? 0 : 1) : (dy == 0 ? 0 : 2), ky1 = py == 0 ? (dy == 0 ? 0 : 2) : (dy == 0 ? 1 : 2);
         const int kx0 = px == 0 ? (dx == 0 ? 0 : 1) : (dx == 0 ? 0 : 2), kx1 = px == 0 ? (dx == 0 ? 0 : 2) : (dx == 0 ? 1 : 2);
-        const int cog = cb * WSU_COB + co;
+        const int cog = cb * WSU_COB + wsu_slot_channel(co);
         float v[16], r[16];
 #pragma unroll
         for (int e = 0; e < 16; ++e) v[e] = 0.f;
@@ -542,14 +562,14 @@
 struct UFormat {
     const char* pack; const char* fwd;
     void (*pack_kernel)(const float*, const float*, char*, float*, int, int, int, int); const char* pack_kernel_name;
-    void (*kernel)(const UArgs); const char* kernel_name; const char* lds_name;
+    void (*kernel)(const UArgs); void (*big_kernel)(const UArgs); const char* kernel_name; const char* lds_name;
     int w_s, w_l;
 };
 const UFormat& u_format(int fmt) {
     static const UFormat q = {"conv3x3_up_pack", "conv3x3_up_q", pack_up_low_kernel<WSU_PLANAR_Q>, "pack_up_low_kernel",
-                              conv3x3_qu_kernel<WSU_PLANAR_Q>, "conv3x3_qu_kernel", "conv3x3_qu", W_S, W_L};
+                              conv3x3_qu_kernel<WSU_PLANAR_Q>, conv3x3_qu_kernel<WSU_PLANAR_Q | FMT_BIG>, "conv3x3_qu_kernel", "conv3x3_qu", W_S, W_L};
     static const UFormat h = {"conv3x3_up_pack_h", "conv3x3_up_h", pack_up_low_kernel<WSU_PLANAR_H>, "pack_up_low_kernel<H>",
-                              conv3x3_qu_kernel<WSU_PLANAR_H>, "conv3x3_qu_kernel<H>", "conv3x3_qu<H>", W_S_H, W_L_H};
+                              conv3x3_qu_kernel<WSU_PLANAR_H>, conv3x3_qu_kernel<WSU_PLANAR_H | FMT_BIG>, "conv3x3_qu_kernel<H>", "conv3x3_qu<H>", W_S_H, W_L_H};
     return fmt == WSU_PLANAR_H ? h : q;
 }
 
@@ -593,13 +613,16 @@
     a.ntiles = (int)nt;
     const int ncu = wsu_cu_count(who);
     if (!ncu) return WSU_ERR_HIP;
-    static bool raised[2] = {false, false};
-    bool& done = raised[fmt == WSU_PLANAR_H];
+    const size_t ychunk = fmt == WSU_PLANAR_H ? wsu_h_chunk_bytes(h, w) : wsu_q_chunk_bytes(h, w);
+    const bool big = 2 * ychunk > 0xFFFFFFF0ull;
+    void (*kernel)(const UArgs) = big ? f.big_kernel : f.kernel;
+    static bool raised[2][2] = {{false, false}, {false, false}};
+    bool& done = raised[fmt == WSU_PLANAR_H][big];
     if (!done) {
-        if (int rc = wsu_raise_lds(f.kernel, LDS_TOTAL, f.lds_name)) return rc;
+        if (int rc = wsu_raise_lds(kernel, LDS_TOTAL, f.lds_name)) return rc;
         done = true;
     }
-    hipLaunchKernelGGL(f.kernel, dim3(a.ntiles < ncu ? a.ntiles : ncu), dim3(NT), LDS_TOTAL, static_cast<hipStream_t>(stream), a);
+    hipLaunchKernelGGL(kernel, dim3(a.ntiles < ncu ? a.ntiles : ncu), dim3(NT), LDS_TOTAL, static_cast<hipStream_t>(stream), a);
     return wsu_check_launch(f.kernel_name);
 }
 
diff --git a/ws_unet_amd/csrc/wsu_device.h b/ws_unet_amd/csrc/wsu_device.h
--- a/ws_unet_amd/csrc/wsu_device.h
+++ b/ws_unet_amd/csrc/wsu_device.h
@@ -43,6 +43,11 @@
 #define WSU_GRAN 4
 #define WSU_COB 64
 __host__ __device__ inline int wsu_chunk_channels(int mode) { return mode == WSU_MODE_BF16 ? 32 : 16; }
+__host__ __device__ constexpr int wsu_row_channel(int row) { return ((row >> 2) & 1) * 16 + (row >> 3) * 4 + (row & 3); }
+__host__ __device__ constexpr int wsu_channel_row(int ch) { return ((ch >> 2) & 3) * 8 + (ch >> 4) * 4 + (ch & 3); }
+__host__ __device__ constexpr int wsu_slot_channel(int row64) { return (row64 & 32) + wsu_row_channel(row64 & 31); }
+static_assert(wsu_row_channel(0) == 0 && wsu_row_channel(4) == 16 && wsu_row_channel(8) == 4 && wsu_row_channel(31) == 31 && wsu_channel_row(16) == 4 &&
+              wsu_channel_row(wsu_row_channel(13)) == 13 && wsu_channel_row(wsu_row_channel(22)) == 22 && wsu_slot_channel(36) == 48, "row map");
 
 __device__ __forceinline__ int wsu_reflect(int i, int n) {
     i = i < 0 ? -i : i;
@@ -222,17 +227,6 @@
     wsu_swap32(xh0, yh0); wsu_swap32(xh1, yh1);
     g = mk_u4(xh0, xh1, yh0, yh1);
 }
-__device__ __forceinline__ float wsu_q4_pre(const f32x4& X, const f32x4& Y, u32x4& g, uint32_t& dhi, uint32_t& dres, uint32_t& sb) {
-    uint32_t xh0, xh1, yh0, yh1;
-    wsu_q4_pre_cvt(X, Y, xh0, xh1, yh0, yh1);
-    float mx = __builtin_fmaxf(__builtin_fmaxf(__builtin_fabsf(X[0]), __builtin_fabsf(X[1])), __builtin_fabsf(X[2]));
-    mx = __builtin_fmaxf(__builtin_fmaxf(mx, __builtin_fabsf(X[3])), __builtin_fabsf(Y[0]));
-    mx = __builtin_fmaxf(__builtin_fmaxf(mx, __builtin_fabsf(Y[1])), __builtin_fabsf(Y[2]));
-    mx = __builtin_fmaxf(mx, __builtin_fabsf(Y[3]));
-    const f32x2 mm = {mx, 0.f};
-    wsu_q4_pre_enc(X, Y, xh0, xh1, yh0, yh1, __builtin_bit_cast(uint32_t, __builtin_convertvector(mm, f16x2)), g, dhi, dres, sb);
-    return mx;
-}
 __device__ __forceinline__ void wsu_q4_pre_bits(const f32x4& X, const f32x4& Y, u32x4& g, uint32_t& dhi, uint32_t& dres, uint32_t& sb) {
     uint32_t xh0, xh1, yh0, yh1;
     wsu_q4_pre_cvt(X, Y, xh0, xh1, yh0, yh1);
@@ -249,22 +243,24 @@
     return mk_u4(__builtin_amdgcn_perm(dhi1, dhi0, 0x05040100u), __builtin_amdgcn_perm(dhi1, dhi0, 0x07060302u),
                  __builtin_amdgcn_perm(dres1, dres0, 0x05040100u), __builtin_amdgcn_perm(dres1, dres0, 0x07060302u));
 }
-__device__ __forceinline__ u32x4 wsu_q4_single(uint32_t dhi, uint32_t dres) {
-    uint32_t ph = dhi, pr = dres;
-    wsu_swap32(dhi, ph); wsu_swap32(dres, pr);
-    return mk_u4(__builtin_amdgcn_perm(ph, dhi, 0x05040100u), __builtin_amdgcn_perm(ph, dhi, 0x07060302u),
-                 __builtin_amdgcn_perm(pr, dres, 0x05040100u), __builtin_amdgcn_perm(pr, dres, 0x07060302u));
-}
 #define WSU_F16_RANGE 65504.f
 __host__ __device__ inline size_t wsu_h_chunk_bytes(int h, int w) { return (size_t)32 * h * w; }
-__device__ __forceinline__ u32x4 wsu_h_granule(const f32x4& X, const f32x4& Y) {
-    const f32x2 xa = {X[0], X[1]}, xb = {X[2], X[3]}, ya = {Y[0], Y[1]}, yb = {Y[2], Y[3]};
-    uint32_t xh0 = __builtin_bit_cast(uint32_t, __builtin_convertvector(xa, f16x2)), xh1 = __builtin_bit_cast(uint32_t, __builtin_convertvector(xb, f16x2));
-    uint32_t yh0 = __builtin_bit_cast(uint32_t, __builtin_convertvector(ya, f16x2)), yh1 = __builtin_bit_cast(uint32_t, __builtin_convertvector(yb, f16x2));
-    wsu_swap32(xh0, yh0); wsu_swap32(xh1, yh1);
-    return mk_u4(xh0, xh1, yh0, yh1);
-}
-__device__ __forceinline__ void wsu_q4_encode16(const f32x4 (&v)[4], u32x4& h0, u32x4& h1, u32x4& q, uint32_t& sb) {
+__device__ __forceinline__ void wsu_h_encode16(const f32x4 (&v)[4], u32x4& h0, u32x4& h1) {
+    uint32_t h[8];
+#pragma unroll
+    for (int k = 0; k < 4; ++k) {
+        const f32x2 a = {v[k][0], v[k][1]}, b = {v[k][2], v[k][3]};
+        h[2 * k] = __builtin_bit_cast(uint32_t, __builtin_convertvector(a, f16x2)); h[2 * k + 1] = __builtin_bit_cast(uint32_t, __builtin_convertvector(b, f16x2));
+    }
+    h0 = mk_u4(h[0], h[1], h[2], h[3]); h1 = mk_u4(h[4], h[5], h[6], h[7]);
+}
+__device__ __forceinline__ void wsu_a_encode16(const f32x4 (&v)[4], u32x4& h0, u32x4& h1, u32x4& lo) {
+    uint32_t h[8], l[4];
+#pragma unroll
+    for (int k = 0; k < 4; ++k) wsu_split4_f16r8(v[k], WSU_F8_XLO_DIV, h[2 * k], h[2 * k + 1], l[k]);
+    h0 = mk_u4(h[0], h[1], h[2], h[3]); h1 = mk_u4(h[4], h[5], h[6], h[7]); lo = mk_u4(l[0], l[1], l[2], l[3]);
+}
+__device__ __forceinline__ void wsu_q4_encode16_with(const f32x4 (&v)[4], uint32_t mb, bool have_mb, u32x4& h0, u32x4& h1, u32x4& q, uint32_t& sb) {
     uint32_t h[8]; float r[16];
 #pragma unroll
     for (int k = 0; k < 4; ++k) {
@@ -274,7 +270,7 @@
         r[4 * k + 2] = wsu_sub_f16_lo(v[k][2], h[2 * k + 1]); r[4 * k + 3] = wsu_sub_f16_hi(v[k][3], h[2 * k + 1]);
     }
     h0 = mk_u4(h[0], h[1], h[2], h[3]); h1 = mk_u4(h[4], h[5], h[6], h[7]);
-    const int e = wsu_q4_block_exp(wsu_f16x16_max_abs_bits(h0, h1));
+    const int e = wsu_q4_block_exp(have_mb ? mb : wsu_f16x16_max_abs_bits(h0, h1));
     const float sc = wsu_pow2f(e), scr = wsu_pow2f(e - 11);
     sb = (uint32_t)(e + 127);
     uint32_t q2 = 0, q3 = 0;
@@ -283,6 +279,22 @@
     q3 = __builtin_amdgcn_cvt_scalef32_pk_fp4_f32(q3, r[8], r[9], scr, 0); q3 = __builtin_amdgcn_cvt_scalef32_pk_fp4_f32(q3, r[10], r[11], scr, 1);
     q3 = __builtin_amdgcn_cvt_scalef32_pk_fp4_f32(q3, r[12], r[13], scr, 2); q3 = __builtin_amdgcn_cvt_scalef32_pk_fp4_f32(q3, r[14], r[15], scr, 3);
     q = mk_u4(wsu_f16x8_to_fp4(h0, sc), wsu_f16x8_to_fp4(h1, sc), q2, q3);
+}
+__device__ __forceinline__ void wsu_q4_encode16(const f32x4 (&v)[4], u32x4& h0, u32x4& h1, u32x4& q, uint32_t& sb) {
+    wsu_q4_encode16_with(v, 0u, false, h0, h1, q, sb);
+}
+__device__ __forceinline__ float wsu_q4_encode16_max(const f32x4 (&v)[4], u32x4& h0, u32x4& h1, u32x4& q, uint32_t& sb) {
+    float mx = __builtin_fmaxf(__builtin_fmaxf(__builtin_fabsf(v[0][0]), __builtin_fabsf(v[0][1])), __builtin_fabsf(v[0][2]));
+    mx = __builtin_fmaxf(__builtin_fmaxf(mx, __builtin_fabsf(v[0][3])), __builtin_fabsf(v[1][0]));
+    mx = __builtin_fmaxf(__builtin_fmaxf(mx, __builtin_fabsf(v[1][1])), __builtin_fabsf(v[1][2]));
+    mx = __builtin_fmaxf(__builtin_fmaxf(mx, __builtin_fabsf(v[1][3])), __builtin_fabsf(v[2][0]));
+    mx = __builtin_fmaxf(__builtin_fmaxf(mx, __builtin_fabsf(v[2][1])), __builtin_fabsf(v[2][2]));
+    mx = __builtin_fmaxf(__builtin_fmaxf(mx, __builtin_fabsf(v[2][3])), __builtin_fabsf(v[3][0]));
+    mx = __builtin_fmaxf(__builtin_fmaxf(mx, __builtin_fabsf(v[3][1])), __builtin_fabsf(v[3][2]));
+    mx = __builtin_fmaxf(mx, __builtin_fabsf(v[3][3]));
+    const f32x2 mm = {mx, 0.f};
+    wsu_q4_encode16_with(v, __builtin_bit_cast(uint32_t, __builtin_convertvector(mm, f16x2)), true, h0, h1, q, sb);
+    return mx;
 }
 __device__ __forceinline__ void wsu_mfma_q4(const u32x4& a, const u32x4& b, int scale_a, int scale_b, f32x16& acc) {
     const i32x8 av = {(int)a.x, (int)a.y, (int)a.z, (int)a.w, 0, 0, 0, 0}, bv = {(int)b.x, (int)b.y, (int)b.z, (int)b.w, 0, 0, 0, 0};
```
